# oasys-mas/free-range-zoo

Measured on NVIDIA B200. Metric: env-steps/sec, higher is better.
Workload: dtype int32+f32

## Files before the change

### __graft_entry__.py

```python
import os
import subprocess
import sys

ROOT = os.path.dirname(os.path.abspath(__file__))
if ROOT not in sys.path:
    sys.path.insert(0, ROOT)


def build() -> None:
    from oracle.build_ref import build_ref
    build_ref()
    from free_range_zoo_b200 import _build
    path = _build.build(verbose=False)
    assert os.path.exists(path), path
    from free_range_zoo_b200 import _lib
    lib = _lib.library()
    missing = [name for header in ('frz.h', 'frz_obs.h', 'frz_autoreset.h') for name in _lib.exported_symbols(header)
               if not hasattr(lib, name)]
    if missing:
        raise RuntimeError(f'libfrz.so does not export {missing}')
    import free_range_zoo_b200.envs.wildfire_v0


def smoke() -> None:
    import numpy as np
    import torch

    from free_range_zoo_b200 import presets
    from free_range_zoo_b200.envs import wildfire_v0
    from oracle.wildfire import WildfireOracle

    B, steps = 64, 3
    config = presets.wildfire_large()
    env = wildfire_v0.parallel_env(parallel_envs=B, max_steps=10, configuration=config, device=torch.device('cuda:0'))
    env.reset(seed=0)
    oracle = WildfireOracle(config, B, 10)
    oracle.reset()
    rng = np.random.default_rng(0)
    for _ in range(steps):
        counts = oracle.agent_task_count
        k = np.minimum((rng.random(counts.shape) * (counts + 1)).astype(np.int64), counts)
        actions = np.stack([k, np.where(k == counts, -1, 0)], axis=2).astype(np.int32)
        u_field = rng.random((3, B, 10, 10), dtype=np.float32)
        u_agent = rng.random((5, B, 10), dtype=np.float32)
        oracle.step(actions, u_field, u_agent)
        env.unwrapped.inject_uniforms(torch.from_numpy(u_field), torch.from_numpy(u_agent))
        _, rewards, terminations, _, _ = env.step(torch.from_numpy(actions).cuda())
    state = env.state()
    assert np.array_equal(state.fires.cpu().numpy(), oracle.fires)
    assert np.array_equal(state.intensity.cpu().numpy(), oracle.intensity)
    assert np.array_equal(state.equipment.cpu().numpy(), oracle.equipment)
    got = np.stack([rewards[a].cpu().numpy() for a in env.agents], axis=1)
    assert np.allclose(got, oracle.rewards, rtol=1e-5, atol=1e-6)
    print('smoke ok: wildfire 10x10/10 agents, 64 envs x 3 steps bit-exact vs oracle (injected uniforms)')

    from tests import philox_ref
    B, seed = 300, 0xC0FFEE
    env = wildfire_v0.parallel_env(parallel_envs=B, max_steps=10, configuration=config, device=torch.device('cuda:0'))
    env.reset(seed=seed)
    raw = env.unwrapped
    oracle = WildfireOracle(config, B, 10)
    oracle.reset()
    for t in range(steps):
        actions = philox_ref.sampled_actions(7, t, np.arange(B), oracle.agent_task_count)
        raw.sample_actions(7)
        assert np.array_equal(raw._actions.cpu().numpy(), actions)
        oracle.step(actions, *philox_ref.wildfire_uniforms(seed, t, np.arange(B), 10, 10, 10))
        raw.step_all()
    state = raw.state()
    for name in ('fires', 'intensity', 'fuel', 'equipment', 'suppressants', 'capacity'):
        assert np.array_equal(getattr(state, name).cpu().numpy(), getattr(oracle, name)), name
    assert np.array_equal(raw._task_obs.cpu().numpy(), oracle.task_obs)
    assert np.array_equal(raw._agent_task_count.cpu().numpy(), oracle.agent_task_count)
    assert np.allclose(raw._rewards.cpu().numpy(), oracle.rewards, rtol=1e-5, atol=1e-6)
    raw.check_errors()
    print('smoke ok: Philox-mode kernel, 300 envs x 3 steps bit-exact vs oracle on host-Philox uniforms')


if __name__ == '__main__':
    build()
    if len(sys.argv) > 1 and sys.argv[1] == 'smoke':
        smoke()
```

### free_range_zoo_b200/_lib.py

```python
from __future__ import annotations

import ctypes as C
import os

import torch

_HERE = os.path.dirname(os.path.abspath(__file__))
LIBRARY_PATH = os.environ.get('FRZ_LIBRARY') or os.path.join(_HERE, 'csrc', 'libfrz.so')

MAX_AGENTS = 32
MAX_EQUIPMENT = 8
MAX_CAPACITIES = 8
MAX_CELLS = 256
MAX_NODES = 32
MAX_NET_STATES = 16
MAX_PASSENGERS = 64
PAD = -100

FAULT_NAMES = {
    0x1: 'action[:, 0] is not a valid index into the agent\'s task list',
    0x2: 'cybersecurity attack / movement target outside [0, num_nodes)',
    0x4: 'a non-present cybersecurity agent acted while show_bad_actions=False',
    0x8: 'rideshare passenger table overflow',
}


class Control(C.Structure):
    _fields_ = [('seed', C.c_uint64), ('step', C.c_uint64), ('ctas_done', C.c_uint32), ('alive_acc', C.c_uint32),
                ('alive', C.c_uint32), ('error_word', C.c_uint32), ('agents_with_tasks_acc', C.c_uint32),
                ('agents_with_tasks', C.c_uint32), ('reserved', C.c_uint32 * 6)]


WF_FLAGS = dict(suppressant_decrease=0x0001, suppressant_refill=0x0002, tank_switch=0x0004, critical_error=0x0008,
                degrade=0x0010, repair=0x0020, fire_increase=0x0040, fire_decrease=0x0080,
                special_burnout_probability=0x0100, fire_fuel=0x0200)
WF_BURNOUT_SCALED = 0x0400
WF_LOCALIZE_PUTOUTS = 0x0800
WF_SHOW_BAD_ACTIONS = 0x1000
WF_KERNEL_TILES, WF_KERNEL_GROUPS = 0x2000, 0x4000


class WildfireParams(C.Structure):
    _fields_ = [
        ('height', C.c_int32), ('width', C.c_int32), ('num_agents', C.c_int32), ('num_fire_states', C.c_int32),
        ('num_equipment_states', C.c_int32), ('num_capacities', C.c_int32), ('max_steps', C.c_int32),
        ('flags', C.c_uint32), ('env_offset', C.c_int64),
        ('p_increase', C.c_float), ('p_burnout', C.c_float), ('p_decrease', C.c_float), ('decrease_bonus', C.c_float),
        ('p_random_ignition', C.c_float), ('spread_lut', C.c_float * 16),
        ('p_suppressant_decrease', C.c_float), ('p_refill', C.c_float), ('p_repair', C.c_float),
        ('p_degrade', C.c_float), ('p_critical', C.c_float), ('p_tank_switch', C.c_float),
        ('capacity_cum', C.c_float * MAX_CAPACITIES), ('capacity_value', C.c_float * MAX_CAPACITIES),
        ('equipment_capacity_bonus', C.c_float * MAX_EQUIPMENT), ('equipment_power_bonus', C.c_float * MAX_EQUIPMENT),
        ('bad_attack_penalty', C.c_float), ('burnout_penalty', C.c_float), ('termination_reward', C.c_float),
        ('termination_kappa', C.c_float),
        ('agent_y', C.c_int32 * MAX_AGENTS), ('agent_x', C.c_int32 * MAX_AGENTS), ('agent_power', C.c_float * MAX_AGENTS),
    ]


_WF_POINTERS = ('fires', 'intensity', 'fuel', 'suppressants', 'capacity', 'equipment', 'init_fires', 'init_intensity',
                'init_fuel', 'init_suppressants', 'init_capacity', 'init_equipment', 'actions', 'rewards',
                'cumulative_rewards', 'terminated', 'truncated', 'num_moves', 'num_burnouts', 'burnouts', 'putouts',
                'env_task_count', 'agent_task_count', 'action_mask', 'self_obs', 'task_obs', 'cell_reward',
                'cell_ignition', 'range_mask', 'cell_agents', 'control', 'field_uniforms', 'agent_uniforms')


class WildfireBuffers(C.Structure):
    _fields_ = [(name, C.c_void_p) for name in _WF_POINTERS] + [('mask_stride', C.c_int32), ('mask_words', C.c_int32)]


CY_STOCHASTIC_STATE = 0x1
CY_SHOW_BAD_ACTIONS = 0x2
CY_MAX_LUT_BITS = 12


class CyberParams(C.Structure):
    _fields_ = [
        ('num_nodes', C.c_int32), ('num_attackers', C.c_int32), ('num_defenders', C.c_int32), ('num_states', C.c_int32),
        ('max_steps', C.c_int32), ('flags', C.c_uint32), ('env_offset', C.c_int64), ('lut_bits', C.c_int32),
        ('temperature', C.c_float), ('patch_reward', C.c_float), ('bad_action_penalty', C.c_float),
        ('power', C.c_float * MAX_AGENTS), ('persist', C.c_float * MAX_AGENTS), ('returns', C.c_float * MAX_AGENTS),
        ('state_rewards', C.c_float * MAX_NET_STATES), ('criticality', C.c_float * MAX_NODES),
    ]


_CY_POINTERS = ('network_state', 'location', 'presence', 'init_network_state', 'init_location', 'init_presence',
                'actions', 'rewards', 'cumulative_rewards', 'terminated', 'truncated', 'num_moves', 'env_task_count',
                'agent_task_count', 'attacker_self', 'defender_self', 'task_obs', 'monitored', 'score_lut', 'control',
                'network_uniforms', 'agent_uniforms')


class CyberBuffers(C.Structure):
    _fields_ = [(name, C.c_void_p) for name in _CY_POINTERS]


RS_FAST_TRAVEL = 0x1
RS_DIAGONAL_TRAVEL = 0x2
RS_VARIABLE_MOVE_COST = 0x4
RS_WAITING_COSTS = 0x8
RS_KERNEL_TILES, RS_KERNEL_GROUPS = 0x100, 0x200
RS_PASSENGER_COLUMNS = 11
RS_TASK_COLUMNS = 8


class RideshareParams(C.Structure):
    _fields_ = [
        ('num_agents', C.c_int32), ('capacity', C.c_int32), ('schedule_rows', C.c_int32), ('schedule_horizon', C.c_int32),
        ('pool_limit', C.c_int32),
        ('max_steps', C.c_int32), ('flags', C.c_uint32), ('env_offset', C.c_int64), ('wait_limit', C.c_int32 * 3),
        ('long_wait_time', C.c_int32), ('move_cost', C.c_float), ('drop_cost', C.c_float), ('noop_cost', C.c_float),
        ('accept_cost', C.c_float), ('pool_limit_cost', C.c_float), ('general_wait_cost', C.c_float),
        ('long_wait_cost', C.c_float),
    ]


_RS_POINTERS = ('agents', 'passengers', 'init_agents', 'init_passengers', 'init_count', 'schedule', 'schedule_index', 'actions',
                'rewards', 'cumulative_rewards', 'terminated', 'truncated', 'num_moves', 'env_task_count',
                'agent_task_count', 'task_mask', 'self_obs', 'task_obs', 'control')


class RideshareBuffers(C.Structure):
    _fields_ = [(name, C.c_void_p) for name in _RS_POINTERS]


MAX_CHUNKS = 16


class HostStep(C.Structure):
    _fields_ = [('actions', C.c_void_p), ('rewards', C.c_void_p), ('terminated', C.c_void_p), ('truncated', C.c_void_p),
                ('chunk_controls', C.c_void_p), ('streams', C.POINTER(C.c_void_p)), ('chunks', C.c_int32),
                ('action_format', C.c_int32), ('packed_actions', C.c_void_p), ('pipeline', C.c_void_p)]


class GatherArray(C.Structure):
    _fields_ = [('src', C.c_void_p), ('dst', C.c_void_p), ('row_bytes', C.c_int32), ('capacity', C.c_int32),
                ('groups', C.c_int32), ('reserved', C.c_int32)]


class ObsArray(C.Structure):
    _fields_ = [('src', C.c_void_p), ('dst', C.c_void_p), ('host', C.c_void_p), ('kind', C.c_int32), ('src_type', C.c_int32),
                ('dst_type', C.c_int32), ('groups', C.c_int32), ('capacity', C.c_int32), ('src_columns', C.c_int32),
                ('column_first', C.c_int32), ('columns', C.c_int32)]


class ObsDownload(C.Structure):
    _fields_ = [('counts', C.c_void_p), ('offsets', C.c_void_p), ('host_offsets', C.c_void_p), ('scan', C.c_void_p),
                ('scratch', C.c_void_p),
                ('status', C.c_void_p), ('arrays', C.POINTER(ObsArray)), ('array_count', C.c_int32),
                ('mask_groups', C.c_int32)]


class AutoresetRow(C.Structure):
    _fields_ = [('dst', C.c_void_p), ('src', C.c_void_p), ('bytes', C.c_int64)]


AUTORESET_MAX_ROWS = 32


class Autoreset(C.Structure):
    _fields_ = [(name, C.c_void_p) for name in (
        'terminated', 'truncated', 'step_terminated', 'step_truncated', 'done', 'cumulative_rewards', 'episode_return',
        'num_moves', 'episode_length', 'agent_task_count', 'reset_agent_task_count', 'control', 'finished',
        'finished_count', 'scratch')] + [('rows', C.POINTER(AutoresetRow)), ('row_count', C.c_int32),
                                         ('num_agents', C.c_int32)]


OBS_DENSE, OBS_ROWS, OBS_MASK_BITS = 0, 1, 2
OBS_I32, OBS_I16, OBS_I8, OBS_U8, OBS_F32 = 0, 1, 2, 3, 4
HOST_ACTIONS_I32, HOST_ACTIONS_I16, HOST_ACTIONS_I8 = 0, 1, 2
ABI_VERSION = 4


_lib = None


def library() -> C.CDLL:
    global _lib
    if _lib is not None:
        return _lib
    if not os.path.exists(LIBRARY_PATH):
        raise RuntimeError(f'{LIBRARY_PATH} is missing: the B200 engine has no CPU fallback. '
                           'Build it with `python -c "import __graft_entry__ as g; g.build()"`.')
    lib = C.CDLL(LIBRARY_PATH)
    lib.frz_version.restype = C.c_int
    lib.frz_last_error.restype = C.c_char_p
    lib.frz_control_init.argtypes = [C.c_void_p, C.c_uint64, C.c_void_p]
    for name in ('frz_wildfire_step', 'frz_wildfire_refresh'):
        getattr(lib, name).argtypes = [C.POINTER(WildfireParams), C.POINTER(WildfireBuffers), C.c_int32, C.c_void_p]
    lib.frz_wildfire_reset.argtypes = [C.POINTER(WildfireParams), C.POINTER(WildfireBuffers), C.c_int32, C.c_void_p,
                                       C.c_void_p]
    lib.frz_wildfire_sample_actions.argtypes = [C.POINTER(WildfireParams), C.POINTER(WildfireBuffers), C.c_int32,
                                                C.c_uint64, C.c_void_p]
    for name in ('frz_cyber_step', 'frz_cyber_refresh'):
        getattr(lib, name).argtypes = [C.POINTER(CyberParams), C.POINTER(CyberBuffers), C.c_int32, C.c_void_p]
    lib.frz_cyber_reset.argtypes = [C.POINTER(CyberParams), C.POINTER(CyberBuffers), C.c_int32, C.c_void_p, C.c_void_p]
    lib.frz_cyber_sample_actions.argtypes = [C.POINTER(CyberParams), C.POINTER(CyberBuffers), C.c_int32, C.c_uint64,
                                             C.c_void_p]
    for name in ('frz_rideshare_step', 'frz_rideshare_refresh'):
        getattr(lib, name).argtypes = [C.POINTER(RideshareParams), C.POINTER(RideshareBuffers), C.c_int32, C.c_void_p]
    lib.frz_rideshare_reset.argtypes = [C.POINTER(RideshareParams), C.POINTER(RideshareBuffers), C.c_int32, C.c_void_p,
                                        C.c_void_p]
    lib.frz_rideshare_sample_actions.argtypes = [C.POINTER(RideshareParams), C.POINTER(RideshareBuffers), C.c_int32,
                                                 C.c_uint64, C.c_void_p]
    for name, params, buffers in (('frz_wildfire_step_host', WildfireParams, WildfireBuffers),
                                  ('frz_cyber_step_host', CyberParams, CyberBuffers),
                                  ('frz_rideshare_step_host', RideshareParams, RideshareBuffers)):
        getattr(lib, name).argtypes = [C.POINTER(params), C.POINTER(buffers), C.c_int32, C.POINTER(HostStep), C.c_void_p]
    lib.frz_host_slices.argtypes = [C.c_int32, C.c_int32, C.POINTER(C.c_int32)]
    lib.frz_wildfire_tile_random_layout.argtypes = [C.POINTER(WildfireParams), C.POINTER(C.c_uint32), C.POINTER(C.c_int8)]
    lib.frz_gather_live_rows.argtypes = [C.c_void_p, C.c_int32, C.c_void_p, C.c_void_p, C.POINTER(GatherArray), C.c_int32,
                                         C.c_void_p]
    lib.frz_observe_compact.argtypes = [C.POINTER(ObsDownload), C.c_int32, C.c_void_p]
    lib.frz_autoreset.argtypes = [C.POINTER(Autoreset), C.c_int32, C.c_void_p]
    if lib.frz_version() != ABI_VERSION:
        raise RuntimeError(f'libfrz.so ABI version {lib.frz_version()} != {ABI_VERSION}; rebuild the library')
    lib.frz_control_restore.argtypes = [C.c_void_p, C.c_uint64, C.c_uint64, C.c_void_p]
    lib.frz_host_pipeline_create.argtypes = [C.POINTER(C.c_void_p)]
    lib.frz_host_pipeline_destroy.argtypes = [C.c_void_p]
    for name, params in (('frz_wildfire_buffer_bytes', WildfireParams), ('frz_cyber_buffer_bytes', CyberParams),
                         ('frz_rideshare_buffer_bytes', RideshareParams)):
        getattr(lib, name).argtypes = [C.POINTER(params), C.c_int32, C.c_char_p]
        getattr(lib, name).restype = C.c_int64
    _lib = lib
    return lib


def host_slices(parallel_envs: int, chunks: int):
    bounds = (C.c_int32 * (MAX_CHUNKS + 1))()
    count = library().frz_host_slices(parallel_envs, chunks, bounds)
    if count < 0:
        check(-count, 'frz_host_slices')
    return list(bounds[:count + 1])


def check(status: int, what: str = '') -> None:
    if status != 0:
        message = library().frz_last_error().decode()
        raise RuntimeError(f'libfrz {what} failed (status {status}): {message}')


def stream_handle(device: torch.device) -> C.c_void_p:
    return C.c_void_p(torch.cuda.current_stream(device).cuda_stream)


def pointer(tensor: torch.Tensor | None) -> int | None:
    return None if tensor is None else tensor.data_ptr()


def exported_symbols(header: str = 'frz.h'):
    import re
    header = os.path.join(os.path.dirname(_HERE), 'include', header)
    text = open(header).read()
    return sorted(set(re.findall(r'\b(frz_[a-z_]+)\s*\(', text)))
```

### free_range_zoo_b200/csrc/frz_common.cuh

```cuda
#pragma once

#include <cuda_runtime.h>
#include <stdint.h>

#include <vector>

#include "frz.h"

struct FrzHostPipeline {
  int device = -1;
  cudaEvent_t events[1 + 2 * FRZ_MAX_CHUNKS] = {};
  cudaGraph_t graph = nullptr;
  cudaGraphExec_t exec = nullptr;
  std::vector<unsigned char> signature;
  struct ActionCopy {
    cudaGraphNode_t node;
    void* dst;
    size_t offset, bytes;
  };
  std::vector<ActionCopy> action_copies;
  const void* captured_actions = nullptr;
};

namespace frz {

constexpr unsigned kFullMask = 0xffffffffu;
constexpr int kMaxDevices = 64;


void set_error(const char* fmt, ...);
int check_launch(const char* what);

inline int current_device() {
  int device = 0;
  cudaGetDevice(&device);
  return device;
}

inline int sm_count() {
  static int cache[kMaxDevices] = {};
  const int device = current_device();
  int count = (device >= 0 && device < kMaxDevices) ? cache[device] : 0;
  if (count == 0) {
    cudaDeviceGetAttribute(&count, cudaDevAttrMultiProcessorCount, device);
    if (count < 1) count = 1;
    if (device >= 0 && device < kMaxDevices) cache[device] = count;
  }
  return count;
}

template <class Kernel>
int resident_ctas(Kernel kernel, int threads, size_t smem) {
  static int ctas[kMaxDevices] = {};
  static size_t smem_of[kMaxDevices] = {};
  const int device = current_device();
  const bool cacheable = device >= 0 && device < kMaxDevices;
  if (cacheable && ctas[device] > 0 && smem_of[device] == smem) return ctas[device];
  int count = 0;
  cudaOccupancyMaxActiveBlocksPerMultiprocessor(&count, kernel, threads, smem);
  if (count < 1) count = 1;
  if (cacheable) {
    ctas[device] = count;
    smem_of[device] = smem;
  }
  return count;
}

inline int persistent_grid(int work_ctas, int ctas_per_sm) {
  const int cap = sm_count() * ctas_per_sm;
  return work_ctas < cap ? (work_ctas < 1 ? 1 : work_ctas) : cap;
}

int control_broadcast(FrzControl* main_block, FrzControl* chunk_blocks, int count, cudaStream_t stream);
int control_merge(FrzControl* main_block, FrzControl* chunk_blocks, int count, cudaStream_t stream);
cudaEvent_t* pipeline_events(FrzHostPipeline* pipeline);
int widen_actions(const void* packed, int element_bytes, int32_t* actions, size_t count, cudaStream_t stream);


struct Philox {
  uint32_t key0, key1;
  __device__ __forceinline__ Philox(uint64_t seed) : key0(uint32_t(seed)), key1(uint32_t(seed >> 32)) {}

  __device__ __forceinline__ uint4 operator()(uint32_t c0, uint32_t c1, uint32_t c2, uint32_t c3) const {
    uint32_t k0 = key0, k1 = key1;
#pragma unroll
    for (int round = 0; round < 10; ++round) {
      const uint32_t hi0 = __umulhi(0xD2511F53u, c0), lo0 = 0xD2511F53u * c0;
      const uint32_t hi1 = __umulhi(0xCD9E8D57u, c2), lo1 = 0xCD9E8D57u * c2;
      c0 = hi1 ^ c1 ^ k0;
      c1 = lo1;
      c2 = hi0 ^ c3 ^ k1;
      c3 = lo0;
      k0 += 0x9E3779B9u;
      k1 += 0xBB67AE85u;
    }
    return make_uint4(c0, c1, c2, c3);
  }
};

__device__ __forceinline__ float u01(uint32_t bits) { return float(bits >> 8) * 5.9604644775390625e-08f; }

__device__ __forceinline__ int select_bit(uint32_t w, int k) {
  int pos = 0;
#pragma unroll
  for (int span = 16; span >= 1; span >>= 1) {
    const int below = __popc(w & ((1u << span) - 1u));
    if (k >= below) {
      k -= below;
      w >>= span;
      pos += span;
    }
  }
  return pos;
}


__device__ __forceinline__ uint32_t shared_address(const void* pointer) {
  return static_cast<uint32_t>(__cvta_generic_to_shared(pointer));
}
__device__ __forceinline__ uint32_t lds_const(uint32_t address) {
  uint32_t value;
  asm("ld.shared.u32 %0, [%1];" : "=r"(value) : "r"(address));
  return value;
}
__device__ __forceinline__ uint4 lds_const_v4(uint32_t address) {
  uint4 value;
  asm("ld.shared.v4.u32 {%0, %1, %2, %3}, [%4];" : "=r"(value.x), "=r"(value.y), "=r"(value.z), "=r"(value.w) : "r"(address));
  return value;
}
__device__ __forceinline__ uint32_t lds(uint32_t address) {
  uint32_t value;
  asm volatile("ld.shared.u32 %0, [%1];" : "=r"(value) : "r"(address) : "memory");
  return value;
}
__device__ __forceinline__ uint4 lds_v4(uint32_t address) {
  uint4 value;
  asm volatile("ld.shared.v4.u32 {%0, %1, %2, %3}, [%4];"
               : "=r"(value.x), "=r"(value.y), "=r"(value.z), "=r"(value.w) : "r"(address) : "memory");
  return value;
}
__device__ __forceinline__ void sts(uint32_t address, uint32_t value) {
  asm volatile("st.shared.u32 [%0], %1;" : : "r"(address), "r"(value) : "memory");
}

__device__ __forceinline__ void cp_async_4(uint32_t shared_dst, const void* global_src) {
  asm volatile("cp.async.ca.shared.global [%0], [%1], 4;" : : "r"(shared_dst), "l"(global_src) : "memory");
}
__device__ __forceinline__ void cp_async_8(uint32_t shared_dst, const void* global_src) {
  asm volatile("cp.async.ca.shared.global [%0], [%1], 8;" : : "r"(shared_dst), "l"(global_src) : "memory");
}
__device__ __forceinline__ void cp_async_16(uint32_t shared_dst, const void* global_src) {
  asm volatile("cp.async.cg.shared.global [%0], [%1], 16;" : : "r"(shared_dst), "l"(global_src) : "memory");
}
__device__ __forceinline__ void cp_async_commit() { asm volatile("cp.async.commit_group;" : : : "memory"); }
__device__ __forceinline__ void cp_async_wait_all() { asm volatile("cp.async.wait_group 0;" : : : "memory"); }


__device__ __forceinline__ bool elect_one() {
  uint32_t elected;
  asm volatile(
      "{\n"
      ".reg .pred p;\n"
      "elect.sync _|p, 0xffffffff;\n"
      "selp.u32 %0, 1, 0, p;\n"
      "}\n"
      : "=r"(elected));
  return elected != 0u;
}

__device__ __forceinline__ void mbarrier_init(uint32_t barrier, uint32_t arrivals) {
  asm volatile("mbarrier.init.shared::cta.b64 [%0], %1;" : : "r"(barrier), "r"(arrivals) : "memory");
  asm volatile("fence.mbarrier_init.release.cluster;" : : : "memory");
}
__device__ __forceinline__ void mbarrier_expect_bytes(uint32_t barrier, uint32_t bytes) {
  asm volatile("mbarrier.arrive.expect_tx.shared::cta.b64 _, [%0], %1;" : : "r"(barrier), "r"(bytes) : "memory");
}
__device__ __forceinline__ void mbarrier_arrive(uint32_t barrier) {
  asm volatile("mbarrier.arrive.shared::cta.b64 _, [%0];" : : "r"(barrier) : "memory");
}
__device__ __forceinline__ void named_barrier_sync(int id, int threads) {
  asm volatile("bar.sync %0, %1;" : : "r"(id), "r"(threads) : "memory");
}
__device__ __forceinline__ void mbarrier_wait(uint32_t barrier, uint32_t parity) {
  asm volatile(
      "{\n"
      ".reg .pred done;\n"
      "WAIT_LOOP:\n"
      "mbarrier.try_wait.parity.shared::cta.b64 done, [%0], %1;\n"
      "@!done bra WAIT_LOOP;\n"
      "}\n"
      : : "r"(barrier), "r"(parity) : "memory");
}
__device__ __forceinline__ void bulk_load(uint32_t shared_dst, const void* global_src, uint32_t bytes, uint32_t barrier) {
  asm volatile("cp.async.bulk.shared::cluster.global.mbarrier::complete_tx::bytes [%0], [%1], %2, [%3];"
               : : "r"(shared_dst), "l"(global_src), "r"(bytes), "r"(barrier) : "memory");
}
__device__ __forceinline__ void bulk_store(void* global_dst, uint32_t shared_src, uint32_t bytes) {
  asm volatile("cp.async.bulk.global.shared::cta.bulk_group [%0], [%1], %2;"
               : : "l"(global_dst), "r"(shared_src), "r"(bytes) : "memory");
}
__device__ __forceinline__ void bulk_commit() { asm volatile("cp.async.bulk.commit_group;" : : : "memory"); }
__device__ __forceinline__ void bulk_wait_read() { asm volatile("cp.async.bulk.wait_group.read 0;" : : : "memory"); }
template <int pending>
__device__ __forceinline__ void bulk_wait_read_all_but() {
  asm volatile("cp.async.bulk.wait_group.read %0;" : : "n"(pending) : "memory");
}
__device__ __forceinline__ void fence_async_shared() { asm volatile("fence.proxy.async.shared::cta;" : : : "memory"); }


enum Publish { kPublishNothing = 0, kPublishRefresh = 1, kPublishStep = 2 };

__device__ __forceinline__ void finish_launch(FrzControl* control, unsigned alive_bits, unsigned fault_bits,
                                              unsigned agent_bits, int publish) {
  __shared__ unsigned s_alive, s_fault, s_agents;
  if (threadIdx.x == 0) {
    s_alive = 0;
    s_fault = 0;
    s_agents = 0;
  }
  __syncthreads();
  if (alive_bits) atomicOr(&s_alive, alive_bits);
  if (fault_bits) atomicOr(&s_fault, fault_bits);
  if (agent_bits) atomicOr(&s_agents, agent_bits);
  __syncthreads();
  if (threadIdx.x == 0) {
    if (s_alive) atomicOr(&control->alive_acc, s_alive);
    if (s_fault) atomicOr(&control->error_word, s_fault);
    if (s_agents) atomicOr(&control->agents_with_tasks_acc, s_agents);
    __threadfence();
    const unsigned arrived = atomicAdd(&control->ctas_done, 1u) + 1u;
    if (arrived == gridDim.x) {
      __threadfence();
      const unsigned alive = atomicExch(&control->alive_acc, 0u);
      const unsigned agents = atomicExch(&control->agents_with_tasks_acc, 0u);
      if (publish == kPublishStep) {
        control->alive = alive;
        control->step += 1;
      }
      if (publish != kPublishNothing) control->agents_with_tasks = agents;
      if (publish == kPublishRefresh) control->alive = alive;
      control->ctas_done = 0u;
    }
  }
}

}
```

### free_range_zoo_b200/csrc/frz_wildfire.cu

```cuda
#include <cmath>
#include <math_constants.h>

#include "frz_common.cuh"
#include "frz_host.cuh"

namespace frz {
namespace {

#ifndef FRZ_WF_THREADS
#define FRZ_WF_THREADS 256
#endif
constexpr int kThreads = FRZ_WF_THREADS;
enum Mode { kStep = 0, kRefresh = 1 };

template <int NW>
__device__ __forceinline__ uint32_t word_at(const uint32_t (&words)[NW], int index) {
  uint32_t w = words[0];
#pragma unroll
  for (int i = 1; i < NW; ++i) w = (index == i) ? words[i] : w;
  return w;
}

template <int NW>
__device__ __forceinline__ bool bit_at(const uint32_t (&words)[NW], int cell) {
  return (word_at<NW>(words, cell >> 5) >> (cell & 31)) & 1u;
}

template <int G>
__device__ __forceinline__ float group_sum(float v) {
#pragma unroll
  for (int offset = G / 2; offset >= 1; offset >>= 1) v += __shfl_xor_sync(kFullMask, v, offset, G);
  return v;
}

template <int G>
__device__ __forceinline__ int group_sum(int v) {
#pragma unroll
  for (int offset = G / 2; offset >= 1; offset >>= 1) v += __shfl_xor_sync(kFullMask, v, offset, G);
  return v;
}

template <int G>
__device__ __forceinline__ uint32_t group_ballot(bool pred, int group_base, uint32_t group_mask) {
  const uint32_t ballot = __ballot_sync(kFullMask, pred);
  return (G == 32) ? ballot : ((ballot >> group_base) & group_mask);
}

#ifndef FRZ_WF_CELLS_IN_SMEM
#define FRZ_WF_CELLS_IN_SMEM 1
#endif
__host__ __device__ constexpr bool split_geometry(int group, int cells_per_lane) { return group == 16 && cells_per_lane > 4; }
__host__ __device__ constexpr bool cells_in_smem(int group, int cells_per_lane) {
  return FRZ_WF_CELLS_IN_SMEM && split_geometry(group, cells_per_lane);
}
__host__ __device__ constexpr int group_smem_words(int group, int cells_per_lane) {
  const int cells = group * cells_per_lane;
  const int words = cells_in_smem(group, cells_per_lane) ? 8 * cells + 5 * group : 2 * cells;
  return (group == 16 && words % 32 == 0) ? words + 16 : words;
}
__host__ __device__ inline int static_smem_words(int cells, int agents, int states) {
  const int words = (cells + 31) / 32;
  return 4 * cells + states * cells + agents * states * words;
}

template <int G, int CPL, int NW>
__device__ __forceinline__ void assemble_words(const uint32_t (&rows)[CPL], uint32_t (&words)[NW], int group_base,
                                               uint32_t group_mask, uint32_t half_selector) {
  if constexpr (G == 32) {
#pragma unroll
    for (int i = 0; i < CPL; ++i) words[i] = rows[i];
  } else if constexpr (CPL == 1) {
    words[0] = (rows[0] >> group_base) & group_mask;
  } else if constexpr (G == 16) {
#pragma unroll
    for (int w = 0; w < NW; ++w) words[w] = __byte_perm(rows[2 * w], (2 * w + 1 < CPL) ? rows[(2 * w + 1 < CPL) ? 2 * w + 1 : 0] : 0u, half_selector);
  } else {
    static_assert(G == 8 && CPL <= 4, "8-lane groups hold at most 4 cells per lane");
    const uint32_t lo = __byte_perm(rows[0], rows[1], half_selector);
    const uint32_t hi = CPL > 2 ? __byte_perm(rows[2], rows[CPL - 1], half_selector) : 0u;
    uint32_t word = __byte_perm(lo, hi, 0x5410);
    if (CPL == 2) word &= 0xffffu;
    if (CPL == 3) word &= 0xffffffu;
    words[0] = word;
  }
}

template <int NW>
__device__ __forceinline__ void load_range_words(uint32_t address, uint32_t (&words)[NW]) {
  if constexpr (NW == 4) {
    const uint4 v = lds_const_v4(address);
    words[0] = v.x;
    words[1] = v.y;
    words[2] = v.z;
    words[3] = v.w;
  } else {
#pragma unroll
    for (int w = 0; w < NW; ++w) words[w] = lds_const(address + 4u * w);
  }
}

#ifndef FRZ_WF_MIN_BLOCKS
#define FRZ_WF_MIN_BLOCKS 3
#endif

struct Derived {
  uint32_t west_ok[FRZ_MAX_CELLS / 32];
  uint32_t east_ok[FRZ_MAX_CELLS / 32];
  int32_t spare_lanes_feed_agents;
  uint32_t t_increase, t_burnout, t_suppressant_decrease, t_repair, t_critical, t_degrade, t_refill, t_tank_switch;
  int32_t t_capacity_cum[FRZ_MAX_CAPACITIES];
  int32_t almost_state, burned_state;
  int32_t cells;
};

template <int G, int CPL, int MODE, bool INJECTED, bool BULK>
__global__ void __launch_bounds__(kThreads, (G * CPL > 128) ? 1 : FRZ_WF_MIN_BLOCKS)
wildfire_step_kernel(const __grid_constant__ FrzWildfireParams p, const __grid_constant__ FrzWildfireBuffers io,
                     const __grid_constant__ Derived derived, const int B) {
  constexpr int mode = MODE;
  constexpr int kGroupsPerWarp = 32 / G;
  constexpr int kCells = G * CPL;
  constexpr int NW = (kCells + 31) / 32;
  constexpr int kCalls = (2 * CPL + 3) / 4;
  static_assert(G == 32 || G == 16 || CPL <= 4, "8-lane groups hold at most four cells per lane (one mask word)");
  constexpr int RPW = (CPL == 1) ? 1 : 32 / G;
  constexpr int kFullRows = (G == 32) ? CPL / 2 : (CPL - 1);
  extern __shared__ __align__(16) uint32_t smem[];

  const int lane = threadIdx.x & 31;
  const int warp_in_cta = __shfl_sync(kFullMask, int(threadIdx.x >> 5), 0);
  const int sub = lane % G;
  const int group_base = lane - sub;
  const uint32_t group_mask = (G == 32) ? 0xffffffffu : ((1u << G) - 1u);
  uint32_t lane_bit = 1u << sub;
  asm volatile("" : "+r"(lane_bit));
  const auto row_bit = [&](int i) { return lane_bit << ((i % RPW) * G); };
  const uint32_t half_selector = (G == 16) ? ((group_base & 16) ? 0x7632u : 0x5410u)
                                           : (uint32_t(group_base >> 3) | ((4u + uint32_t(group_base >> 3)) << 4));
  const int W = p.width, HW = derived.cells;
  const int A = p.num_agents;
  const int E = p.num_equipment_states;
  const uint32_t flags = p.flags;
  const bool show_bad = flags & FRZ_WF_SHOW_BAD_ACTIONS;
  const bool use_fuel = flags & FRZ_WF_FIRE_FUEL;
  const int mask_words_row = io.mask_stride >> 2;
  const int table_words = io.mask_words;

  constexpr int kYOff = 0, kXOff = kCells, kIgnitionOff = 2 * kCells, kRewardOff = 3 * kCells, kRegionOff = 4 * kCells;
  constexpr int kCellAgentsOff = kRegionOff + (kThreads / 32) * kGroupsPerWarp * group_smem_words(G, CPL);
  constexpr bool kCellsInSmem = cells_in_smem(G, CPL);
  const int range_off = kCellAgentsOff + E * kCells;
  const int attack_off = kRegionOff + (warp_in_cta * kGroupsPerWarp + lane / G) * group_smem_words(G, CPL);
  const int tasks_off = attack_off + kCells;
  const uint32_t s_base = shared_address(smem);
  uint32_t s_cell = s_base + 4u * uint32_t(sub);
  asm volatile("" : "+r"(s_cell));
  uint32_t s_attack = s_base + 4u * uint32_t(attack_off);
  asm volatile("" : "+r"(s_attack));
  const uint32_t s_tasks = s_base + 4u * uint32_t(tasks_off);
  const uint32_t s_range = s_base + 4u * uint32_t(range_off);
  uint32_t* my_state = smem + tasks_off + kCells + sub;
  constexpr bool bulk = BULK;
  static_assert(!BULK || kCellsInSmem, "the bulk path moves the shared-memory state planes");
  const uint32_t s_barriers = s_base + 4u * uint32_t((range_off + A * E * NW + 3) & ~3) + 16u * uint32_t(warp_in_cta);
  const uint32_t s_planes = s_base + 4u * uint32_t(tasks_off + kCells);
  const auto planes_of_group = [&](int g) {
    return s_base + 4u * uint32_t(kRegionOff + (warp_in_cta * kGroupsPerWarp + g) * group_smem_words(G, CPL) + 2 * kCells);
  };
  constexpr uint32_t kBufferBytes = 4u * 3u * kCells;
  const uint32_t s_stage = s_planes + 2u * kBufferBytes + 4u * uint32_t(sub);

  for (int i = threadIdx.x; i < E * kCells; i += kThreads) {
    const int e = i / kCells, c = i - e * kCells;
    smem[kCellAgentsOff + i] = c < HW ? io.cell_agents[e * HW + c] : 0u;
  }
  for (int i = threadIdx.x; i < A * E * NW; i += kThreads) {
    const int row = i / NW, w = i - row * NW;
    smem[range_off + i] = w < table_words ? io.range_mask[row * table_words + w] : 0u;
  }
  for (int c = threadIdx.x; c < kCells; c += kThreads) {
    const int y = c / W, x = c - y * W;
    const bool in_grid = c < HW;
    smem[kYOff + c] = uint32_t(y);
    smem[kXOff + c] = uint32_t(x);
    smem[kIgnitionOff + c] = in_grid ? uint32_t(io.cell_ignition[c]) : 0u;
    smem[kRewardOff + c] = in_grid ? __float_as_uint(io.cell_reward[c]) : 0u;
  }
#pragma unroll
  for (int i = 0; i < CPL; ++i) smem[attack_off + i * G + sub] = 0u;
  if constexpr (kCellsInSmem) {
#pragma unroll
    for (int i = 0; i < 6 * CPL; ++i) my_state[i * G] = 0u;
    if (bulk && lane == 0) {
      mbarrier_init(s_barriers, 1);
      mbarrier_init(s_barriers + 8u, 1);
    }
  }
  __syncthreads();

  FrzControl* const control = io.control;
  const uint64_t step = control->step;
  const uint32_t alive_prev = control->alive;
  const uint32_t agents_with_tasks = control->agents_with_tasks;
  const Philox philox(control->seed);
  const bool skip = (mode == kStep) && ((alive_prev & 3u) != 3u);

  const bool is_agent = sub < A;
  const float base_power = is_agent ? p.agent_power[sub] : 0.f;
  const float agent_yf = is_agent ? float(p.agent_y[sub]) : 0.f;
  const float agent_xf = is_agent ? float(p.agent_x[sub]) : 0.f;

  unsigned alive_bits = 0, faults = 0, agent_bits = 0;

  if (!skip) {
    const int groups_per_cta = (kThreads / 32) * kGroupsPerWarp;
    const int first_env0 = (blockIdx.x * (kThreads / 32) + warp_in_cta) * kGroupsPerWarp;
    const uint32_t row_bytes = 4u * uint32_t(HW);
    const auto fetch_state = [&](int pair, uint32_t into) {
      const uint32_t buffer = __shfl_sync(kFullMask, into, 0);
      if (elect_one()) {
        const uint32_t barrier = s_barriers + 8u * buffer;
        mbarrier_expect_bytes(barrier, uint32_t(kGroupsPerWarp) * 3u * row_bytes);
#pragma unroll
        for (int g = 0; g < kGroupsPerWarp; ++g) {
          const size_t at = size_t(min(pair + g, B - 1)) * size_t(HW);
          const uint32_t planes = planes_of_group(g) + kBufferBytes * buffer;
          bulk_load(planes, io.fires + at, row_bytes, barrier);
          bulk_load(planes + 4u * kCells, io.intensity + at, row_bytes, barrier);
          bulk_load(planes + 8u * kCells, io.fuel + at, row_bytes, barrier);
        }
      }
      if (is_agent) {
        const uint32_t at = uint32_t(min(pair + lane / G, B - 1)) * uint32_t(A) + uint32_t(sub);
        cp_async_4(s_stage, io.suppressants + at);
        cp_async_4(s_stage + 4u * G, io.capacity + at);
        cp_async_4(s_stage + 8u * G, io.equipment + at);
        if (mode == kStep) cp_async_8(s_stage + 12u * G + 4u * uint32_t(sub), io.actions + 2u * at);
      }
      cp_async_commit();
    };
    uint32_t buffer = 0u, parities = 0u;
    if constexpr (kCellsInSmem) {
      if (bulk && first_env0 < B) fetch_state(first_env0, 0u);
    }
    for (int env0 = first_env0; env0 < B; env0 += gridDim.x * groups_per_cta) {
      const int env = env0 + lane / G;
      const bool valid = (G == 32) || env < B;
      const int e = valid ? env : B - 1;
      const uint32_t cell_row = uint32_t(e) * uint32_t(HW);
      const uint32_t agent_at = uint32_t(e) * uint32_t(A) + uint32_t(sub);
      int* const fires_row = io.fires + cell_row;
      int* const inten_row = io.intensity + cell_row;
      int* const fuel_row = io.fuel + cell_row;

      int cell_regs[3][kCellsInSmem ? 1 : CPL] = {};
      const auto cell = [&](int plane, int i) -> int {
        if constexpr (kCellsInSmem) return int(my_state[plane * kCells + i * G]);
        else return cell_regs[plane][i];
      };
      const auto set_cell = [&](int plane, int i, int value) {
        if constexpr (kCellsInSmem) my_state[plane * kCells + i * G] = uint32_t(value);
        else cell_regs[plane][i] = value;
      };
      uint32_t litw[NW], rows[CPL];
      if constexpr (bulk) {
        mbarrier_wait(s_barriers + 8u * buffer, (parities >> buffer) & 1u);
        parities ^= 1u << buffer;
#pragma unroll
        for (int i = 0; i < CPL; ++i) rows[i] = __ballot_sync(kFullMask, cell(0, i) > 0);
      } else {
#pragma unroll
        for (int i = 0; i < CPL; ++i) {
          const int c = i * G + sub;
          const bool in_grid = i < kFullRows || c < HW;
          const int f = in_grid ? fires_row[c] : 0;
          set_cell(0, i, f);
          set_cell(1, i, in_grid ? inten_row[c] : 0);
          set_cell(2, i, in_grid ? fuel_row[c] : 0);
          rows[i] = __ballot_sync(kFullMask, f > 0);
        }
      }
      float supp = 0.f, cap = 0.f;
      int equip = 0;
      int2 staged_action = make_int2(0, -1);
      if constexpr (bulk) {
        cp_async_wait_all();
        if (is_agent) {
          supp = __uint_as_float(lds(s_stage));
          cap = __uint_as_float(lds(s_stage + 4u * G));
          equip = min(max(int(lds(s_stage + 8u * G)), 0), E - 1);
          if (mode == kStep) {
            staged_action.x = int(lds(s_stage + 12u * G + 4u * uint32_t(sub)));
            staged_action.y = int(lds(s_stage + 12u * G + 4u * uint32_t(sub) + 4u));
          }
        }
      } else if (is_agent) {
        supp = io.suppressants[agent_at];
        cap = io.capacity[agent_at];
        equip = min(max(io.equipment[agent_at], 0), E - 1);
      }

      int n_before = 0;
      assemble_words<G, CPL, NW>(rows, litw, group_base, group_mask, half_selector);
#pragma unroll
      for (int w = 0; w < NW; ++w) n_before += __popc(litw[w]);
      if (mode != kStep) n_before = HW;

      float reward = 0.f, cumulative = 0.f;
      int moves = 0, total_burnouts = 0, n_burned = 0, n_putout = 0;
      bool terminated = false, truncated = false;

      const auto prefetch_next = [&]() {
        if constexpr (kCellsInSmem) {
          const int next_env0 = env0 + gridDim.x * groups_per_cta;
          if (bulk && next_env0 < B) {
            if (lane == 0) bulk_wait_read();
            fetch_state(next_env0, buffer ^ 1u);
          }
        }
      };
      if (mode != kStep) prefetch_next();

      if (mode == kStep) {
        int act_k = 0, act_id = -1;
        if (is_agent) {
          const int2 act = bulk ? staged_action : reinterpret_cast<const int2*>(io.actions)[agent_at];
          act_k = act.x;
          act_id = act.y;
          cumulative = io.cumulative_rewards[agent_at];
        }
        moves = io.num_moves[e];
        total_burnouts = io.num_burnouts[e];
        const bool was_terminated = io.terminated[e] != 0;

        const bool refill = is_agent && act_id == -1;
        int target = -1;
        bool bad = false;
        if (is_agent && !refill && ((agents_with_tasks >> sub) & 1u)) {
          uint32_t availw[NW];
          load_range_words<NW>(s_range + 4u * uint32_t((sub * E + equip) * NW), availw);
#pragma unroll
          for (int w = 0; w < NW; ++w) availw[w] = supp > 0.f ? (litw[w] & availw[w]) : 0u;
          int k = act_k, found = -1, base_bit = 0;
          uint32_t chosen = 0u;
          bool hit = false;
          if (k >= 0) {
#pragma unroll
            for (int w = 0; w < NW; ++w) {
              const uint32_t choices = show_bad ? litw[w] : availw[w];
              const int count = __popc(choices);
              if (!hit) {
                if (k < count) {
                  hit = true;
                  chosen = choices;
                  base_bit = 32 * w;
                } else {
                  k -= count;
                }
              }
            }
          }
          if (hit) found = base_bit + select_bit(chosen, k);
          if (found < 0) faults |= FRZ_FAULT_BAD_TASK_INDEX;
          else if (show_bad && !bit_at<NW>(availw, found)) bad = true;
          else target = found;
        }
        const bool user = target >= 0;
        const float power = base_power + p.equipment_power_bonus[equip];

        {
          const uint32_t key = user ? (uint32_t(group_base) << 16 | uint32_t(target)) : (0x80000000u | uint32_t(lane));
          uint32_t peers = __match_any_sync(kFullMask, key);
          if (!user) peers = 0u;
          float total = 0.f;
          while (__any_sync(kFullMask, peers != 0u)) {
            const int source = (__ffs(peers) - 1) & 31;
            const float theirs = __shfl_sync(kFullMask, power, source);
            if (peers != 0u) total = __fadd_rn(total, theirs);
            peers &= peers - 1u;
          }
          if (user) sts(s_attack + 4u * uint32_t(target), __float_as_uint(total));
          __syncwarp();
        }

        constexpr bool kSplit = !INJECTED && split_geometry(G, CPL) && 2 * ((CPL + 3) / 4) == kCalls;
        constexpr int kCallsA = kSplit ? kCalls / 2 : kCalls;
        const auto grow_word = [](int i) { return kSplit ? i : 2 * i; };
        const auto spread_word = [](int i) { return kSplit ? 4 * kCallsA + i : 2 * i + 1; };
        float ua[5], uf[INJECTED ? 3 * CPL : 1];
        uint32_t ka[5];
        uint32_t bits[4 * kCalls];
        const bool inject_agent = INJECTED && io.agent_uniforms != nullptr;
        const bool inject_field = INJECTED && io.field_uniforms != nullptr;
        const uint32_t env_lo = uint32_t(p.env_offset + e), env_hi = uint32_t(uint64_t(p.env_offset + e) >> 32);
        const uint32_t step_lo = uint32_t(step), step_hi = uint32_t(step >> 32) ^ env_hi;
        const auto draw = [&](int first_call, int last_call) {
#pragma unroll
          for (int k = first_call; k < last_call; ++k) {
            const uint4 r = philox(env_lo, step_lo, uint32_t(k * G + sub), step_hi);
            bits[4 * k] = r.x;
            bits[4 * k + 1] = r.y;
            bits[4 * k + 2] = r.z;
            bits[4 * k + 3] = r.w;
          }
        };
        if (!inject_field || !inject_agent) draw(0, kCallsA);
        if constexpr (INJECTED) {
          const size_t plane = size_t(B) * HW;
#pragma unroll
          for (int i = 0; i < CPL; ++i) {
            const int c = i * G + sub;
            if (inject_field) {
#pragma unroll
              for (int ev = 0; ev < 3; ++ev) uf[3 * i + ev] = c < HW ? io.field_uniforms[ev * plane + cell_row + c] : 1.f;
            } else {
              uf[3 * i] = uf[3 * i + 1] = u01(bits[grow_word(i)]);
              uf[3 * i + 2] = u01(bits[spread_word(i)]);
            }
          }
        }
        const auto field_uniform = [&](int i, int event) -> float {
          if constexpr (INJECTED) return uf[3 * i + event];
          else return u01(bits[event == 2 ? spread_word(i) : grow_word(i)]);
        };

        const auto agent_phase = [&]() {
          if (inject_agent) {
#pragma unroll
            for (int ev = 0; ev < 5; ++ev)
              ua[ev] = is_agent ? io.agent_uniforms[(size_t(ev) * B + e) * A + sub] : 1.f;
          } else {
            uint32_t words[4];
            bool have_words = false;
            constexpr int kSpareOwn = 4 * kCalls - 2 * CPL;
            constexpr int kOwnA = kSplit ? CPL : 2 * CPL, kOwnB = kSplit ? 4 * kCallsA + CPL : 2 * CPL + 1;
            if constexpr (CPL > 1) {
              if (derived.spare_lanes_feed_agents) {
                const int first = group_base + ((G - 1 - sub) & (G - 1)), second = group_base + ((G - 1 - A - sub) & (G - 1));
                const uint32_t a = __shfl_sync(kFullMask, bits[grow_word(CPL - 1)], first);
                const uint32_t b = __shfl_sync(kFullMask, bits[spread_word(CPL - 1)], first);
                if constexpr (kSpareOwn == 2) {
                  words[0] = bits[kOwnA < 4 * kCalls ? kOwnA : 0];
                  words[1] = bits[kOwnB < 4 * kCalls ? kOwnB : 0];
                  words[2] = a;
                  words[3] = b;
                } else {
                  words[0] = a;
                  words[1] = b;
                  words[2] = __shfl_sync(kFullMask, bits[grow_word(CPL - 1)], second);
                  words[3] = __shfl_sync(kFullMask, bits[spread_word(CPL - 1)], second);
                }
                have_words = true;
              }
            }
            if (!have_words) {
              const uint4 r = philox(env_lo, step_lo, 0x80000000u | uint32_t(sub), step_hi);
              words[0] = r.x;
              words[1] = r.y;
              words[2] = r.z;
              words[3] = r.w;
            }
            if constexpr (INJECTED) {
              ua[0] = ua[2] = u01(words[0]);
              ua[1] = u01(words[1]);
              ua[3] = u01(words[2]);
              ua[4] = u01(words[3]);
            } else {
              ka[0] = ka[2] = words[0] >> 8;
              ka[1] = words[1] >> 8;
              ka[3] = words[2] >> 8;
              ka[4] = words[3] >> 8;
            }
          }
          const auto happens = [&](int ev, float p_event, uint32_t t_event) -> bool {
            if constexpr (INJECTED) return ua[ev] < p_event;
            else return ka[ev] < t_event;
          };

          const bool decrease = user && happens(0, p.p_suppressant_decrease, derived.t_suppressant_decrease);
          supp = fmaxf(decrease ? __fadd_rn(supp, -1.f) : supp, 0.f);
          {
            const bool pristine = equip == E - 1, damaged = equip == 0;
            const bool wearable = pristine || !damaged;
            const bool repairs = damaged && happens(1, p.p_repair, derived.t_repair);
            const bool critical = pristine && happens(1, p.p_critical, derived.t_critical);
            const bool degrades = wearable && happens(1, p.p_degrade, derived.t_degrade) && !critical;
            if (repairs) equip = E - 1;
            if (critical) equip = 0;
            if (degrades) equip -= 1;
          }
          const bool increased = refill && happens(2, p.p_refill, derived.t_refill);
          if (increased) supp = __fadd_rn(cap, p.equipment_capacity_bonus[max(equip, 0)]);
          if (__any_sync(kFullMask, increased)) {
            int pick = 0;
#pragma unroll
            for (int i = 0; i < FRZ_MAX_CAPACITIES; ++i) {
              if constexpr (INJECTED) pick += ua[3] > p.capacity_cum[i] ? 1 : 0;
              else pick += int(ka[3]) > derived.t_capacity_cum[i] ? 1 : 0;
            }
            pick = min(pick, p.num_capacities - 1);
            const bool switches = increased && happens(4, p.p_tank_switch, derived.t_tank_switch);
            const float extra = __fadd_rn(supp, -cap);
            if (switches) {
              cap = p.capacity_value[pick];
              supp = __fadd_rn(cap, extra);
            }
          }
        };
        if constexpr (!kSplit) agent_phase();

        uint32_t burned_bits = 0, putout_bits = 0;
        uint32_t burnw[NW];
#pragma unroll
        for (int i = 0; i < CPL; ++i) {
          const float attack = __uint_as_float(lds(s_attack + 4u * uint32_t(i * G + sub)));
          int f = cell(0, i), it = cell(1, i);
          const bool burning = f > 0 && it > 0;
          const float diff = __fadd_rn(f > 0 ? float(f) : 0.f, -attack);
          const bool unmet = burning && diff > 0.f;
          bool grow;
          float u_down;
          if constexpr (INJECTED) {
            u_down = field_uniform(i, 1);
            grow = unmet && field_uniform(i, 0) < (it == derived.almost_state ? p.p_burnout : p.p_increase);
          } else {
            const uint32_t k24 = bits[grow_word(i)] >> 8;
            u_down = float(k24) * 5.9604644775390625e-08f;
            grow = unmet && (it == derived.almost_state ? k24 < derived.t_burnout : k24 < derived.t_increase);
          }
          it += grow ? 1 : 0;
          const bool burned = grow && it >= derived.burned_state;
          const bool met = burning && !burned && diff <= 0.f;
          const float prob_down = fminf(fmaxf(__fadd_rn(p.p_decrease, __fmul_rn(-diff, p.decrease_bonus)), 0.f), 1.f);
          const bool shrink = met && u_down < prob_down;
          it -= shrink ? 1 : 0;
          const bool put = shrink && it <= 0;
          if (burned || put) {
            const int fuel = cell(2, i) - 1;
            set_cell(2, i, burned ? max(fuel, 0) : fuel);
            f = -f;
          }
          burned_bits |= uint32_t(burned) << i;
          putout_bits |= uint32_t(put) << i;
          if (!kCellsInSmem || burned || put) set_cell(0, i, f);
          if (!kCellsInSmem || grow || shrink) set_cell(1, i, it);
          rows[i] = __ballot_sync(kFullMask, burning && !burned && !put);
        }
        assemble_words<G, CPL, NW>(rows, burnw, group_base, group_mask, half_selector);
        __syncwarp();
        if (user) sts(s_attack + 4u * uint32_t(target), 0u);

        if constexpr (kSplit) draw(kCallsA, kCalls);
        prefetch_next();
#pragma unroll
        for (int w = 0; w < NW; ++w) {
          int f[RPW], it[RPW];
          bool unlit[RPW], any_unlit = false;
#pragma unroll
          for (int r = 0; r < RPW; ++r) {
            const int i = w * RPW + r;
            unlit[r] = false;
            if (i < CPL) {
              f[r] = cell(0, i);
              it[r] = cell(1, i);
              unlit[r] = f[r] < 0 && it[r] == 0 && (!use_fuel || cell(2, i) > 0);
              any_unlit = any_unlit || unlit[r];
            }
          }
          if (__any_sync(kFullMask, any_unlit)) {
            const uint32_t cur = burnw[w];
            const uint32_t prev = w > 0 ? burnw[w > 0 ? w - 1 : 0] : 0u;
            const uint32_t next = w + 1 < NW ? burnw[w + 1 < NW ? w + 1 : 0] : 0u;
            uint32_t north, south;
            if (W < 32) {
              north = __funnelshift_l(prev, cur, W);
              south = __funnelshift_r(cur, next, W);
            } else {
              const int q = W >> 5, r = W & 31;
              const auto word_or_zero = [&](int v) { return (v >= 0 && v < NW) ? word_at<NW>(burnw, v) : 0u; };
              north = __funnelshift_l(word_or_zero(w - q - 1), word_or_zero(w - q), r);
              south = __funnelshift_r(word_or_zero(w + q), word_or_zero(w + q + 1), r);
            }
            const uint32_t west = __funnelshift_l(prev, cur, 1) & derived.west_ok[w];
            const uint32_t east = __funnelshift_r(cur, next, 1) & derived.east_ok[w];
#pragma unroll
            for (int r = 0; r < RPW; ++r) {
              const int i = w * RPW + r;
              if (i < CPL) {
                const uint32_t my_bit = row_bit(i);
                float prob = 0.f;
                if (north & my_bit) prob = p.spread_lut[1];
                if (west & my_bit) prob = __fadd_rn(prob, p.spread_lut[2]);
                if (east & my_bit) prob = __fadd_rn(prob, p.spread_lut[4]);
                if (south & my_bit) prob = __fadd_rn(prob, p.spread_lut[8]);
                prob = __fadd_rn(prob, p.p_random_ignition);
                if (unlit[r] && field_uniform(i, 2) < prob) {
                  f[r] = -f[r];
                  it[r] = int(lds_const(s_cell + 4u * (kIgnitionOff + i * G)));
                  if (kCellsInSmem) {
                    set_cell(0, i, f[r]);
                    set_cell(1, i, it[r]);
                  }
                }
              }
            }
          }
#pragma unroll
          for (int r = 0; r < RPW; ++r) {
            const int i = w * RPW + r;
            if (i < CPL) {
              if (!kCellsInSmem) {
                set_cell(0, i, f[r]);
                set_cell(1, i, it[r]);
              }
              rows[i] = __ballot_sync(kFullMask, f[r] > 0);
            }
          }
        }
        assemble_words<G, CPL, NW>(rows, litw, group_base, group_mask, half_selector);

        if constexpr (kSplit) agent_phase();

        if constexpr (G == 32) {
          n_burned = __reduce_add_sync(kFullMask, __popc(burned_bits));
          n_putout = __reduce_add_sync(kFullMask, __popc(putout_bits));
        } else {
          n_burned = group_sum<G>(__popc(burned_bits));
          n_putout = group_sum<G>(__popc(putout_bits));
        }
        float put_total = 0.f, burn_total = 0.f;
        uint32_t putw[NW];
#pragma unroll
        for (int w = 0; w < NW; ++w) putw[w] = 0u;
        const bool localize = flags & FRZ_WF_LOCALIZE_PUTOUTS, scaled = flags & FRZ_WF_BURNOUT_SCALED;
        if (__any_sync(kFullMask, n_putout != 0) && !localize) {
          float my_put_reward = 0.f;
#pragma unroll
          for (int i = 0; i < CPL; ++i)
            if ((putout_bits >> i) & 1u) my_put_reward += __uint_as_float(lds_const(s_cell + 4u * (kRewardOff + i * G)));
          put_total = group_sum<G>(my_put_reward);
        }
        if (__any_sync(kFullMask, n_putout != 0) && localize) {
#pragma unroll
          for (int i = 0; i < CPL; ++i) rows[i] = __ballot_sync(kFullMask, (putout_bits >> i) & 1u);
          assemble_words<G, CPL, NW>(rows, putw, group_base, group_mask, half_selector);
        }
        if (__any_sync(kFullMask, n_burned != 0) && scaled) {
          float my_burn_reward = 0.f;
#pragma unroll
          for (int i = 0; i < CPL; ++i)
            if ((burned_bits >> i) & 1u) my_burn_reward += __uint_as_float(lds_const(s_cell + 4u * (kRewardOff + i * G)));
          burn_total = group_sum<G>(my_burn_reward);
        }
        const float penalty_total =
            (flags & FRZ_WF_BURNOUT_SCALED) ? -burn_total : __fmul_rn(p.burnout_penalty, float(n_burned));
        uint32_t any_lit = 0;
#pragma unroll
        for (int w = 0; w < NW; ++w) any_lit |= litw[w];
        bool dead = any_lit == 0;
        if (use_fuel && __any_sync(kFullMask, dead)) {
          int my_fuel = 0;
#pragma unroll
          for (int i = 0; i < CPL; ++i) my_fuel += cell(2, i);
          const int fuel_left = group_sum<G>(my_fuel);
          dead = dead && fuel_left <= 0;
        }
        if (dead) {
#pragma unroll
          for (int i = 0; i < CPL; ++i) set_cell(0, i, 0);
#pragma unroll
          for (int w = 0; w < NW; ++w) litw[w] = 0;
        }
        const bool newly = !was_terminated && dead;
        terminated = was_terminated || dead;
        reward = bad ? p.bad_attack_penalty : 0.f;
        float gain = put_total;
        if (flags & FRZ_WF_LOCALIZE_PUTOUTS)
          gain = (target >= 0 && bit_at<NW>(putw, target)) ? __uint_as_float(lds_const(s_base + 4u * uint32_t(kRewardOff + target))) : 0.f;
        reward = __fadd_rn(reward, __fadd_rn(gain, penalty_total));
        if (newly) {
          const float penalty = __fmul_rn(p.termination_kappa, logf(__fadd_rn(float(total_burnouts), 1.f)));
          reward = __fadd_rn(reward, fmaxf(__fadd_rn(p.termination_reward, -penalty), 0.f));
        }
        total_burnouts += n_burned;
        moves += 1;
        truncated = moves >= p.max_steps;
        cumulative = __fadd_rn(cumulative, reward);
        if (valid) alive_bits |= (terminated ? 0u : 1u) | (truncated ? 0u : 2u);
      } else if (valid) {
        alive_bits |= (io.terminated[e] ? 0u : 1u) | (io.truncated[e] ? 0u : 2u);
      }

      if constexpr (G != 32) {
        if (!valid) {
          n_before = 0;
#pragma unroll
          for (int w = 0; w < NW; ++w) litw[w] = 0u;
        }
      }
      int n_lit = 0;
#pragma unroll
      for (int w = 0; w < NW; ++w) n_lit += __popc(litw[w]);
      const int n_rows = max(n_lit, n_before);

      int n_avail = 0;
      if (is_agent && supp > 0.f) {
        uint32_t reach[NW];
        load_range_words<NW>(s_range + 4u * uint32_t((sub * E + max(equip, 0)) * NW), reach);
#pragma unroll
        for (int w = 0; w < NW; ++w) n_avail += __popc(litw[w] & reach[w]);
      }
      uint32_t fighters[CPL];
#pragma unroll
      for (int i = 0; i < CPL; ++i) fighters[i] = 0u;
      for (int q = 0; q < E; ++q) {
        const uint32_t ready = group_ballot<G>(is_agent && supp > 0.f && equip == q, group_base, group_mask);
#pragma unroll
        for (int i = 0; i < CPL; ++i) fighters[i] |= lds_const(s_cell + 4u * uint32_t(kCellAgentsOff + q * kCells + i * G)) & ready;
      }
      int4* const task_rows = reinterpret_cast<int4*>(io.task_obs);
      {
        int rank = 0;
#pragma unroll
        for (int i = 0; i < CPL; ++i) {
          const uint32_t word = litw[i / RPW], my_bit = row_bit(i);
          if (i > 0 && i % RPW == 0) rank += __popc(litw[i > 0 ? i / RPW - 1 : 0]);
          if (word & my_bit) {
            const int t = rank + __popc(word & (my_bit - 1u));
            sts(s_tasks + 4u * uint32_t(t), fighters[i]);
            task_rows[cell_row + uint32_t(t)] = make_int4(int(lds_const(s_cell + 4u * (kYOff + i * G))), int(lds_const(s_cell + 4u * (kXOff + i * G))),
                                      cell(0, i), cell(1, i));
          }
        }
      }
      const int quads = (n_rows + 3) >> 2;
      const int quads_warp = __reduce_max_sync(kFullMask, quads);
      for (int first = n_lit; first < 4 * quads; first += G) {
        const int t = first + sub;
        if (t < 4 * quads) {
          sts(s_tasks + 4u * uint32_t(t), 0u);
          if (t < n_before) task_rows[cell_row + uint32_t(t)] = make_int4(FRZ_PAD, FRZ_PAD, FRZ_PAD, FRZ_PAD);
        }
      }
      __syncwarp();

      if (valid) {
        uint32_t* const mask_words = reinterpret_cast<uint32_t*>(io.action_mask);
        const uint32_t mask_env = uint32_t(env) * uint32_t(A) * uint32_t(mask_words_row);
        const int span_shift = min(32 - __clz(max(quads_warp, 1) - 1), (G == 32) ? 5 : (G == 16) ? 4 : 3);
        const int span = 1 << span_shift, slots = G >> span_shift;
        const int slot = sub >> span_shift, quad_in_span = sub & (span - 1);
        for (int first = 0; first < quads; first += span) {
          const int q = first + quad_in_span;
          if (q < quads) {
            const uint4 m = lds_v4(s_tasks + 16u * uint32_t(q));
            constexpr int kPlanes = G / 8;
            uint32_t at = mask_env + uint32_t(slot * mask_words_row + q);
            const uint32_t stride = uint32_t(slots * mask_words_row);
            int a = slot;
#pragma unroll
            for (int k = 0; k < kPlanes; ++k) {
              if (k > 0 && 8 * k >= A) break;
              const uint32_t selector = uint32_t(k | ((4 + k) << 4));
              const uint32_t plane = __byte_perm(__byte_perm(m.x, m.y, selector), __byte_perm(m.z, m.w, selector), 0x5410);
              const int end = min(A, 8 * k + 8);
              for (; a < end; a += slots, at += stride) mask_words[at] = (plane >> (a & 7)) & 0x01010101u;
            }
          }
        }

        if (is_agent) {
          io.agent_task_count[agent_at] = n_avail;
          if (n_avail > 0) agent_bits |= lane_bit;
          reinterpret_cast<float4*>(io.self_obs)[agent_at] =
              make_float4(agent_yf, agent_xf, base_power, supp);
        }
        if (sub == 0) io.env_task_count[env] = n_lit;

        if (mode == kStep) {
          if (!bulk) {
#pragma unroll
            for (int i = 0; i < CPL; ++i) {
              const int c = i * G + sub;
              if (i < kFullRows || c < HW) {
                fires_row[c] = cell(0, i);
                inten_row[c] = cell(1, i);
                fuel_row[c] = cell(2, i);
              }
            }
          }
          if (is_agent) {
            io.suppressants[agent_at] = supp;
            io.capacity[agent_at] = cap;
            io.equipment[agent_at] = equip;
            io.rewards[agent_at] = reward;
            io.cumulative_rewards[agent_at] = cumulative;
          }
          if (sub == 0) {
            io.terminated[env] = terminated;
            io.truncated[env] = truncated;
            io.num_moves[env] = moves;
            io.num_burnouts[env] = total_burnouts;
            io.burnouts[env] = n_burned;
            io.putouts[env] = n_putout;
          }
        }
      }
      if constexpr (kCellsInSmem) {
        if (bulk) {
          if (mode == kStep) {
            fence_async_shared();
            __syncwarp();
            const uint32_t from = __shfl_sync(kFullMask, buffer, 0);
            if (lane == 0) {
#pragma unroll
              for (int g = 0; g < kGroupsPerWarp; ++g) {
                if (env0 + g < B) {
                  const size_t at = size_t(env0 + g) * size_t(HW);
                  const uint32_t planes = planes_of_group(g) + kBufferBytes * from;
                  bulk_store(io.fires + at, planes, row_bytes);
                  bulk_store(io.intensity + at, planes + 4u * kCells, row_bytes);
                  bulk_store(io.fuel + at, planes + 8u * kCells, row_bytes);
                }
              }
              bulk_commit();
            }
          }
          buffer ^= 1u;
          my_state = smem + tasks_off + kCells + sub + buffer * (3 * kCells);
        }
      }
      __syncwarp();
    }
    if constexpr (kCellsInSmem) {
      if (bulk && lane == 0) bulk_wait_read();
    }
  }
  finish_launch(control, alive_bits, faults, agent_bits,
                skip ? kPublishNothing : (mode == kStep ? kPublishStep : kPublishRefresh));
}


__global__ void wildfire_restore_kernel(const FrzWildfireParams p, const FrzWildfireBuffers io, const int B,
                                        const uint8_t* __restrict__ env_mask) {
  const int HW = p.height * p.width, A = p.num_agents;
  const int per_env = HW > A ? HW : A;
  const size_t total = size_t(B) * per_env;
  for (size_t i = size_t(blockIdx.x) * blockDim.x + threadIdx.x; i < total; i += size_t(gridDim.x) * blockDim.x) {
    const int env = int(i / per_env), j = int(i % per_env);
    if (env_mask != nullptr && !env_mask[env]) continue;
    if (j < HW) {
      const size_t at = size_t(env) * HW + j;
      io.fires[at] = io.init_fires[at];
      io.intensity[at] = io.init_intensity[at];
      io.fuel[at] = io.init_fuel[at];
    }
    if (j < A) {
      const size_t at = size_t(env) * A + j;
      io.suppressants[at] = io.init_suppressants[at];
      io.capacity[at] = io.init_capacity[at];
      io.equipment[at] = io.init_equipment[at];
      io.rewards[at] = 0.f;
      io.cumulative_rewards[at] = 0.f;
    }
    if (j == 0) {
      io.terminated[env] = 0;
      io.truncated[env] = 0;
      io.num_moves[env] = 0;
      io.num_burnouts[env] = 0;
      io.burnouts[env] = 0;
      io.putouts[env] = 0;
    }
  }
}

__global__ void wildfire_sample_kernel(const FrzWildfireParams p, const FrzWildfireBuffers io, const int B,
                                       const uint64_t sampler_seed) {
  const int A = p.num_agents;
  const Philox philox(sampler_seed);
  const uint64_t step = io.control->step;
  const bool show_bad = p.flags & FRZ_WF_SHOW_BAD_ACTIONS;
  const int total = B * A;
  for (int i = blockIdx.x * blockDim.x + threadIdx.x; i < total; i += gridDim.x * blockDim.x) {
    const int env = i / A, agent = i - env * A;
    const int n = show_bad ? io.env_task_count[env] : io.agent_task_count[i];
    const uint64_t genv = uint64_t(p.env_offset + env);
    const uint4 r = philox(uint32_t(genv), uint32_t(step), 0xC0000000u | uint32_t(agent), uint32_t(step >> 32) ^ uint32_t(genv >> 32));
    const int k = min(int(u01(r.x) * float(n + 1)), n);
    reinterpret_cast<int2*>(const_cast<int32_t*>(io.actions))[i] = make_int2(k, k == n ? -1 : 0);
  }
}

#ifndef FRZ_WF_HALF_WARP_CELLS
#define FRZ_WF_HALF_WARP_CELLS 128
#endif

struct Geometry {
  int group, cells_per_lane;
};

bool pick_geometry(const FrzWildfireParams& p, Geometry* g) {
  const int HW = p.height * p.width, A = p.num_agents;
  if (A < 1 || A > FRZ_MAX_AGENTS || HW < 1 || HW > FRZ_MAX_CELLS) return false;
  if (HW <= 8 && A <= 8) *g = {8, 1};
  else if (HW <= 32 && A <= 8) *g = {8, (HW + 7) / 8};
  else if (HW <= 16 && A <= 16) *g = {16, 1};
  else if (HW <= FRZ_WF_HALF_WARP_CELLS && A <= 16) *g = {16, (HW + 15) / 16};
  else if (HW <= 32) *g = {32, 1};
  else if (HW <= 64) *g = {32, 2};
  else if (HW <= 128) *g = {32, 4};
  else *g = {32, 8};
  return true;
}

void fold_configuration(const FrzWildfireParams& in, int group, int cells_per_lane, FrzWildfireParams* out, Derived* derived) {
  *out = in;
  const uint32_t flags = in.flags;
  const auto clamp01 = [](float v) { return v < 0.f ? 0.f : (v > 1.f ? 1.f : v); };
  if (!(flags & FRZ_WF_STOCH_SUPPRESSANT_DECREASE)) out->p_suppressant_decrease = 2.f;
  if (!(flags & FRZ_WF_STOCH_REFILL)) out->p_refill = 2.f;
  if (!(flags & FRZ_WF_STOCH_TANK_SWITCH)) out->p_tank_switch = 2.f;
  if (!(flags & FRZ_WF_CRITICAL_ERROR)) out->p_critical = -1.f;
  if (!(flags & FRZ_WF_STOCH_DEGRADE)) out->p_degrade = 2.f;
  if (!(flags & FRZ_WF_STOCH_REPAIR)) out->p_repair = 2.f;
  out->p_increase = (flags & FRZ_WF_STOCH_FIRE_INCREASE) ? clamp01(in.p_increase) : 1.f;
  out->p_burnout = clamp01((flags & FRZ_WF_SPECIAL_BURNOUT) ? in.p_burnout : in.p_increase);
  if (!(flags & FRZ_WF_STOCH_FIRE_DECREASE)) {
    out->p_decrease = 2.f;
    out->decrease_bonus = 0.f;
  }
  for (int i = in.num_capacities; i < FRZ_MAX_CAPACITIES; ++i) out->capacity_cum[i] = INFINITY;
  const int H = in.height, W = in.width, HW = H * W;
  for (int w = 0; w < FRZ_MAX_CELLS / 32; ++w) derived->west_ok[w] = derived->east_ok[w] = 0u;
  for (int c = 0; c < HW; ++c) {
    const int x = c % W;
    if (x > 0) derived->west_ok[c >> 5] |= 1u << (c & 31);
    if (x < W - 1) derived->east_ok[c >> 5] |= 1u << (c & 31);
  }
  {
    const auto below = [](float probability) {
      const double scaled = std::ceil(double(probability) * 16777216.0);
      return uint32_t(scaled < 0.0 ? 0.0 : (scaled > 16777216.0 ? 16777216.0 : scaled));
    };
    derived->t_increase = below(out->p_increase);
    derived->t_burnout = below(out->p_burnout);
    derived->t_suppressant_decrease = below(out->p_suppressant_decrease);
    derived->t_repair = below(out->p_repair);
    derived->t_critical = below(out->p_critical);
    derived->t_degrade = below(out->p_degrade);
    derived->t_refill = below(out->p_refill);
    derived->t_tank_switch = below(out->p_tank_switch);
    for (int i = 0; i < FRZ_MAX_CAPACITIES; ++i) {
      const double scaled = std::floor(double(out->capacity_cum[i]) * 16777216.0);
      derived->t_capacity_cum[i] = std::isnan(scaled) ? (1 << 24) : int32_t(scaled < -1.0 ? -1.0 : (scaled > 16777216.0 ? 16777216.0 : scaled));
    }
    derived->almost_state = in.num_fire_states - 2;
    derived->burned_state = in.num_fire_states - 1;
    derived->cells = in.height * in.width;
  }
  derived->spare_lanes_feed_agents = 0;
  if (cells_per_lane > 1) {
    const int last_row_cells = HW - group * (cells_per_lane - 1);
    const int spare_lanes = group - (last_row_cells > 0 ? last_row_cells : 0);
    const int calls = (2 * cells_per_lane + 3) / 4, spare_own = 4 * calls - 2 * cells_per_lane;
    const int lanes_needed = spare_own == 2 ? in.num_agents : 2 * in.num_agents;
    derived->spare_lanes_feed_agents = lanes_needed <= spare_lanes ? 1 : 0;
  }
}

#include "frz_wildfire_tile.cuh"

template <int MAXA, int MODE, bool INJECTED>
int launch_tiles(const FrzWildfireParams& caller_params, const FrzWildfireBuffers& io, int B, const Geometry& g,
                 cudaStream_t stream) {
  FrzWildfireParams p;
  Derived derived;
  fold_configuration(caller_params, g.group, g.cells_per_lane, &p, &derived);
  const SmallRandomLayout layout = small_random_layout(p.height * p.width, p.num_agents, g.group, g.cells_per_lane,
                                                       derived.spare_lanes_feed_agents != 0);
  const size_t smem = size_t(small_tile(p.height * p.width, p.num_agents).total) * sizeof(uint32_t);
  auto kernel = wildfire_tile_kernel<MAXA, MODE, INJECTED>;
  if (smem > 48 * 1024 && cudaFuncSetAttribute(kernel, cudaFuncAttributeMaxDynamicSharedMemorySize, int(smem)) != cudaSuccess)
    return check_launch("wildfire tile shared memory");
  cudaFuncSetAttribute(kernel, cudaFuncAttributePreferredSharedMemoryCarveout, cudaSharedmemCarveoutMaxShared);
  const int tiles = (B + 31) / 32;
  const int resident = sm_count() * resident_ctas(kernel, 32, smem);
  const int rounds = (tiles + resident - 1) / resident;
  const int grid = (tiles + rounds - 1) / rounds;
  kernel<<<grid, 32, smem, stream>>>(p, io, derived, layout, B);
  return check_launch("wildfire_tile_kernel");
}

template <int MAXA>
int launch_tiles_mode(const FrzWildfireParams& p, const FrzWildfireBuffers& io, int B, int mode, const Geometry& g,
                      cudaStream_t stream) {
  if (mode != kStep) return launch_tiles<MAXA, kRefresh, false>(p, io, B, g, stream);
  if (io.field_uniforms != nullptr || io.agent_uniforms != nullptr) return launch_tiles<MAXA, kStep, true>(p, io, B, g, stream);
  return launch_tiles<MAXA, kStep, false>(p, io, B, g, stream);
}

template <int G, int CPL, int MODE, bool INJECTED, bool BULK>
int launch_variant(const FrzWildfireParams& caller_params, const FrzWildfireBuffers& io, int B, cudaStream_t stream) {
  FrzWildfireParams p;
  Derived derived;
  fold_configuration(caller_params, G, CPL, &p, &derived);
  const int groups_per_cta = (kThreads / 32) * (32 / G);
  const size_t smem = (size_t(static_smem_words(G * CPL, p.num_agents, p.num_equipment_states)) +
                       size_t(groups_per_cta) * group_smem_words(G, CPL)) * sizeof(uint32_t) +
                      (BULK ? 16 + 16 * (kThreads / 32) : 0);
  auto kernel = wildfire_step_kernel<G, CPL, MODE, INJECTED, BULK>;
  if (smem > 48 * 1024) {
    if (cudaFuncSetAttribute(kernel, cudaFuncAttributeMaxDynamicSharedMemorySize, int(smem)) != cudaSuccess)
      return check_launch("wildfire smem attribute");
  }
  const int grid = persistent_grid((B + groups_per_cta - 1) / groups_per_cta, resident_ctas(kernel, kThreads, smem));
  kernel<<<grid, kThreads, smem, stream>>>(p, io, derived, B);
  return check_launch("wildfire_step_kernel");
}

template <int G, int CPL, bool BULK>
int launch_mode(const FrzWildfireParams& p, const FrzWildfireBuffers& io, int B, int mode, cudaStream_t stream) {
  if (mode != kStep) return launch_variant<G, CPL, kRefresh, false, BULK>(p, io, B, stream);
  if (io.field_uniforms != nullptr || io.agent_uniforms != nullptr) return launch_variant<G, CPL, kStep, true, BULK>(p, io, B, stream);
  return launch_variant<G, CPL, kStep, false, BULK>(p, io, B, stream);
}

template <int G, int CPL>
int launch_step(const FrzWildfireParams& p, const FrzWildfireBuffers& io, int B, int mode, cudaStream_t stream) {
  if constexpr (cells_in_smem(G, CPL)) {
    const uintptr_t bases = reinterpret_cast<uintptr_t>(io.fires) | reinterpret_cast<uintptr_t>(io.intensity) |
                            reinterpret_cast<uintptr_t>(io.fuel);
    if ((p.height * p.width) % 4 == 0 && bases % 16 == 0) return launch_mode<G, CPL, true>(p, io, B, mode, stream);
  }
  return launch_mode<G, CPL, false>(p, io, B, mode, stream);
}

int dispatch(const FrzWildfireParams* p, const FrzWildfireBuffers* io, int B, int mode, void* stream) {
  if (p == nullptr || io == nullptr || io->control == nullptr || io->fires == nullptr || io->cell_agents == nullptr ||
      io->range_mask == nullptr) {
    set_error("frz_wildfire: NULL params / buffers");
    return FRZ_ERR_NULL;
  }
  Geometry g;
  if (B <= 0 || !pick_geometry(*p, &g) || p->num_equipment_states < 1 || p->num_equipment_states > FRZ_MAX_EQUIPMENT ||
      p->num_capacities < 1 || p->num_capacities > FRZ_MAX_CAPACITIES || io->mask_stride % 4 != 0 ||
      io->mask_stride < p->height * p->width) {
    set_error("frz_wildfire: unsupported shape B=%d H=%d W=%d A=%d E=%d", B, p->height, p->width, p->num_agents,
              p->num_equipment_states);
    return FRZ_ERR_SHAPE;
  }
  {
    const uint64_t cells = uint64_t(B) * uint64_t(p->height * p->width);
    const uint64_t mask_words = uint64_t(B) * uint64_t(p->num_agents) * uint64_t(io->mask_stride / 4);
    if (cells >= (1ull << 32) || mask_words >= (1ull << 32)) {
      set_error("frz_wildfire: B=%d is too large for one launch (arrays exceed 2^32 elements); shard the batch", B);
      return FRZ_ERR_SHAPE;
    }
  }
  cudaStream_t s = static_cast<cudaStream_t>(stream);
  if (small_grid(*p) && g.group == 8 &&
      ((p->flags & FRZ_WF_KERNEL_TILES) ||
       (!(p->flags & FRZ_WF_KERNEL_GROUPS) && tiny_grid(*p) && B >= kSmallTileMinimumBatch))) {
    return p->num_agents <= 4 ? launch_tiles_mode<4>(*p, *io, B, mode, g, s) : launch_tiles_mode<8>(*p, *io, B, mode, g, s);
  }
  if (g.group == 8) {
    switch (g.cells_per_lane) {
      case 1: return launch_step<8, 1>(*p, *io, B, mode, s);
      case 2: return launch_step<8, 2>(*p, *io, B, mode, s);
      case 3: return launch_step<8, 3>(*p, *io, B, mode, s);
      default: return launch_step<8, 4>(*p, *io, B, mode, s);
    }
  }
  if (g.group == 16) {
    switch (g.cells_per_lane) {
      case 1: return launch_step<16, 1>(*p, *io, B, mode, s);
      case 2: return launch_step<16, 2>(*p, *io, B, mode, s);
      case 3: return launch_step<16, 3>(*p, *io, B, mode, s);
      case 4: return launch_step<16, 4>(*p, *io, B, mode, s);
      case 5: return launch_step<16, 5>(*p, *io, B, mode, s);
      case 6: return launch_step<16, 6>(*p, *io, B, mode, s);
      case 7: return launch_step<16, 7>(*p, *io, B, mode, s);
      default: return launch_step<16, 8>(*p, *io, B, mode, s);
    }
  }
  switch (g.cells_per_lane) {
    case 1: return launch_step<32, 1>(*p, *io, B, mode, s);
    case 2: return launch_step<32, 2>(*p, *io, B, mode, s);
    case 4: return launch_step<32, 4>(*p, *io, B, mode, s);
    default: return launch_step<32, 8>(*p, *io, B, mode, s);
  }
}

}
}

extern "C" {

int frz_wildfire_step(const FrzWildfireParams* params, const FrzWildfireBuffers* io, int32_t parallel_envs, void* stream) {
  if (io != nullptr && io->actions == nullptr) {
    frz::set_error("frz_wildfire_step: actions is NULL");
    return FRZ_ERR_NULL;
  }
  return frz::dispatch(params, io, parallel_envs, frz::kStep, stream);
}

int frz_wildfire_step_host(const FrzWildfireParams* params, const FrzWildfireBuffers* io, int32_t parallel_envs,
                           const FrzHostStep* host, void* stream) {
  if (params == nullptr || io == nullptr || io->actions == nullptr || io->control == nullptr || io->rewards == nullptr) {
    frz::set_error("frz_wildfire_step_host: NULL params / buffers");
    return FRZ_ERR_NULL;
  }
  if (io->field_uniforms != nullptr || io->agent_uniforms != nullptr) {
    frz::set_error("frz_wildfire_step_host: injected uniforms are not supported on the pipelined host path");
    return FRZ_ERR_UNSUPPORTED;
  }
  const size_t HW = size_t(params->height) * params->width, A = size_t(params->num_agents);
  const frz::HostArrays arrays{io->actions, io->rewards, io->terminated, io->truncated, io->control, params->num_agents,
                                 params, sizeof(FrzWildfireParams), io, sizeof(FrzWildfireBuffers)};
  return frz::run_host_pipeline(
      "frz_wildfire_step_host", host, arrays, parallel_envs, static_cast<cudaStream_t>(stream),
      [&](int first, int count, FrzControl* control, cudaStream_t slice_stream) {
        FrzWildfireParams p = *params;
        p.env_offset += first;
        FrzWildfireBuffers slice = *io;
        const size_t e = size_t(first);
        slice.fires += e * HW;
        slice.intensity += e * HW;
        slice.fuel += e * HW;
        slice.suppressants += e * A;
        slice.capacity += e * A;
        slice.equipment += e * A;
        slice.actions += e * A * 2;
        slice.rewards += e * A;
        slice.cumulative_rewards += e * A;
        slice.terminated += e;
        slice.truncated += e;
        slice.num_moves += e;
        slice.num_burnouts += e;
        slice.burnouts += e;
        slice.putouts += e;
        slice.env_task_count += e;
        slice.agent_task_count += e * A;
        slice.action_mask += e * A * size_t(io->mask_stride);
        slice.self_obs += e * A * 4;
        slice.task_obs += e * HW * 4;
        slice.control = control;
        return frz::dispatch(&p, &slice, count, frz::kStep, slice_stream);
      });
}

int frz_wildfire_tile_random_layout(const FrzWildfireParams* params, uint32_t* streams, int8_t* destinations) {
  frz::Geometry g;
  if (params == nullptr || streams == nullptr || destinations == nullptr) {
    frz::set_error("frz_wildfire_tile_random_layout: NULL argument");
    return -FRZ_ERR_NULL;
  }
  if (!frz::pick_geometry(*params, &g) || !frz::small_grid(*params) || g.group != 8) {
    frz::set_error("frz_wildfire_tile_random_layout: H=%d W=%d A=%d is not a small grid", params->height, params->width,
                   params->num_agents);
    return -FRZ_ERR_SHAPE;
  }
  FrzWildfireParams folded;
  frz::Derived derived;
  frz::fold_configuration(*params, g.group, g.cells_per_lane, &folded, &derived);
  const frz::SmallRandomLayout layout = frz::small_random_layout(
      params->height * params->width, params->num_agents, g.group, g.cells_per_lane, derived.spare_lanes_feed_agents != 0);
  for (int i = 0; i < layout.calls; ++i) {
    streams[i] = layout.stream[i];
    for (int j = 0; j < 4; ++j) destinations[4 * i + j] = layout.dest[i][j];
  }
  return layout.calls;
}

int frz_wildfire_refresh(const FrzWildfireParams* params, const FrzWildfireBuffers* io, int32_t parallel_envs,
                         void* stream) {
  return frz::dispatch(params, io, parallel_envs, frz::kRefresh, stream);
}

int frz_wildfire_reset(const FrzWildfireParams* params, const FrzWildfireBuffers* io, int32_t parallel_envs,
                       const uint8_t* env_mask, void* stream) {
  if (params == nullptr || io == nullptr || io->init_fires == nullptr || io->control == nullptr) {
    frz::set_error("frz_wildfire_reset: NULL params / buffers");
    return FRZ_ERR_NULL;
  }
  if (parallel_envs <= 0) {
    frz::set_error("frz_wildfire_reset: parallel_envs=%d", parallel_envs);
    return FRZ_ERR_SHAPE;
  }
  const int HW = params->height * params->width;
  const size_t total = size_t(parallel_envs) * (HW > params->num_agents ? HW : params->num_agents);
  const int grid = frz::persistent_grid(int((total + 255) / 256 < (1u << 20) ? (total + 255) / 256 : (1u << 20)), 16);
  frz::wildfire_restore_kernel<<<grid, 256, 0, static_cast<cudaStream_t>(stream)>>>(*params, *io, parallel_envs, env_mask);
  const int status = frz::check_launch("wildfire_restore_kernel");
  if (status != FRZ_OK) return status;
  return frz::dispatch(params, io, parallel_envs, frz::kRefresh, stream);
}

int frz_wildfire_sample_actions(const FrzWildfireParams* params, const FrzWildfireBuffers* io, int32_t parallel_envs,
                                uint64_t sampler_seed, void* stream) {
  if (params == nullptr || io == nullptr || io->actions == nullptr || io->control == nullptr) {
    frz::set_error("frz_wildfire_sample_actions: NULL params / buffers");
    return FRZ_ERR_NULL;
  }
  const int total = parallel_envs * params->num_agents;
  const int grid = frz::persistent_grid((total + 255) / 256, 8);
  frz::wildfire_sample_kernel<<<grid, 256, 0, static_cast<cudaStream_t>(stream)>>>(*params, *io, parallel_envs, sampler_seed);
  return frz::check_launch("wildfire_sample_kernel");
}

}
```

### free_range_zoo_b200/envs/wildfire/env/wildfire.py

```python
from __future__ import annotations

import ctypes
from typing import Any, Callable, Dict, List, Optional, Tuple

import numpy as np
import torch

from free_range_zoo_b200 import _lib
from free_range_zoo_b200.envs.wildfire.env.structures.state import WildfireState
from free_range_zoo_b200.utils.containers import (LazyDict, ObservationDict, jagged_from_padded,
                                                  jagged_indices_from_mask)
from free_range_zoo_b200.utils.conversions import batched_aec_to_batched_parallel
from free_range_zoo_b200.utils import compact
from free_range_zoo_b200.utils.env import AutoresetRows, BatchedAECEnv
from free_range_zoo_b200.utils.spaces import BatchedActionSpace, Space


def parallel_env(wrappers: List[Callable] = [], **kwargs):
    env = raw_env(**kwargs)
    for wrapper in wrappers:
        env = wrapper(env)
    return batched_aec_to_batched_parallel(env)


def env(wrappers: List[Callable] = [], **kwargs):
    environment = raw_env(**kwargs)
    for wrapper in wrappers:
        environment = wrapper(environment)
    return environment


def _np(tensor, dtype):
    return np.ascontiguousarray(torch.as_tensor(tensor).detach().cpu().numpy().astype(dtype))


def spread_lut(weights) -> np.ndarray:
    w = _np(weights, np.float32).reshape(3, 3)
    taps = (w[0, 1], w[1, 0], w[1, 2], w[2, 1])
    lut = np.zeros(16, dtype=np.float32)
    for pattern in range(16):
        acc = np.float32(0.0)
        for bit, tap in enumerate(taps):
            if pattern >> bit & 1:
                acc = np.float32(acc + tap)
        lut[pattern] = acc
    return lut


def flatten_configuration(config, max_steps, show_bad_actions: bool, env_offset: int = 0):
    fc, ac, rc, sc = config.fire_config, config.agent_config, config.reward_config, config.stochastic_config
    H, W = int(config.grid_height), int(config.grid_width)
    A = int(ac.agents.shape[0])
    equipment_states = _np(ac.equipment_states, np.float32)
    E = equipment_states.shape[0]
    capacities = _np(ac.possible_capacities, np.float32)
    if H * W > _lib.MAX_CELLS or A > _lib.MAX_AGENTS or E > _lib.MAX_EQUIPMENT or len(capacities) > _lib.MAX_CAPACITIES:
        raise ValueError(f'wildfire configuration exceeds the engine limits: H*W={H * W} (<= {_lib.MAX_CELLS}), '
                         f'agents={A} (<= {_lib.MAX_AGENTS}), equipment states={E}, capacities={len(capacities)}')

    p = _lib.WildfireParams()
    p.height, p.width, p.num_agents = H, W, A
    p.num_fire_states = int(fc.num_fire_states)
    p.num_equipment_states = E
    p.num_capacities = len(capacities)
    p.max_steps = 2**31 - 1 if max_steps is None else int(max_steps)
    flags = 0
    for name, bit in _lib.WF_FLAGS.items():
        if getattr(sc, name):
            flags |= bit
    if rc.burnout_penalty_scaled:
        flags |= _lib.WF_BURNOUT_SCALED
    if rc.localize_putouts:
        flags |= _lib.WF_LOCALIZE_PUTOUTS
    if show_bad_actions:
        flags |= _lib.WF_SHOW_BAD_ACTIONS
    p.flags = flags
    p.env_offset = env_offset
    p.p_increase = fc.intensity_increase_probability
    p.p_burnout = fc.burnout_probability
    p.p_decrease = fc.intensity_decrease_probability
    p.decrease_bonus = fc.extra_power_decrease_bonus
    p.p_random_ignition = config.fire_random_spread_weight
    p.spread_lut[:] = spread_lut(config.fire_spread_weights).tolist()
    p.p_suppressant_decrease = ac.suppressant_decrease_probability
    p.p_refill = ac.suppressant_refill_probability
    p.p_repair = ac.repair_probability
    p.p_degrade = ac.degrade_probability
    p.p_critical = ac.critical_error_probability
    p.p_tank_switch = ac.tank_switch_probability
    cumulative = np.cumsum(_np(ac.capacity_probabilities, np.float32), dtype=np.float32)
    for i in range(len(capacities)):
        p.capacity_cum[i] = cumulative[i]
        p.capacity_value[i] = capacities[i]
    for e in range(E):
        p.equipment_capacity_bonus[e] = equipment_states[e, 0]
        p.equipment_power_bonus[e] = equipment_states[e, 1]
    p.bad_attack_penalty = rc.bad_attack_penalty
    p.burnout_penalty = rc.burnout_penalty
    p.termination_reward = rc.termination_reward
    p.termination_kappa = rc.termination_kappa
    positions = _np(ac.agents, np.int32)
    power = _np(ac.fire_reduction_power, np.float32)
    for a in range(A):
        p.agent_y[a], p.agent_x[a], p.agent_power[a] = int(positions[a, 0]), int(positions[a, 1]), float(power[a])

    words = (H * W + 31) // 32
    ys, xs = np.divmod(np.arange(H * W), W)
    attack_range = _np(ac.attack_range, np.float32)
    range_mask = np.zeros((A, E, words), dtype=np.uint32)
    for a in range(A):
        chebyshev = np.maximum(np.abs(positions[a, 0] - ys), np.abs(positions[a, 1] - xs)).astype(np.float32)
        for e in range(E):
            reach = np.float32(attack_range[a] + equipment_states[e, 2])
            for c in np.nonzero(chebyshev <= reach)[0]:
                range_mask[a, e, c >> 5] |= np.uint32(1 << (c & 31))
    return p, _np(rc.fire_rewards, np.float32).reshape(-1), _np(fc.ignition_temp, np.int32).reshape(-1), range_mask


def compact_bounds(config) -> Dict[str, int]:
    H, W, fc = int(config.grid_height), int(config.grid_width), config.fire_config
    max_fire_type = max(int(fc.max_fire_type), int(torch.as_tensor(fc.fire_types).abs().max()))
    return dict(task_obs=max(H - 1, W - 1, max_fire_type, int(fc.num_fire_states) - 1),
                agent_task_count=H * W)


def transpose_range_mask(range_mask: np.ndarray, cells: int) -> np.ndarray:
    agents, states, _ = range_mask.shape
    cell_agents = np.zeros((states, cells), dtype=np.uint32)
    for a in range(agents):
        for e in range(states):
            for c in range(cells):
                if int(range_mask[a, e, c >> 5]) >> (c & 31) & 1:
                    cell_agents[e, c] |= np.uint32(1 << a)
    return cell_agents


class raw_env(BatchedAECEnv):

    metadata = {"render.modes": ["human", "rgb_array"], "name": "wildfire_v0", "is_parallelizable": True,
                "render_fps": 2}

    @torch.no_grad()
    def __init__(self, *args, observe_other_suppressant: bool = False, observe_other_power: bool = False,
                 show_bad_actions: bool = False, step_kernel: str = 'auto', **kwargs) -> None:
        super().__init__(*args, **kwargs)
        if step_kernel not in ('auto', 'tiles', 'groups'):
            raise ValueError(f"step_kernel must be 'auto', 'tiles' or 'groups', not {step_kernel!r}")
        self._step_kernel = step_kernel
        self.observe_other_suppressant = observe_other_suppressant
        self.observe_other_power = observe_other_power
        self.show_bad_actions = show_bad_actions

        A = int(self.agent_config.agents.shape[0])
        self.possible_agents = tuple(f"firefighter_{i}" for i in range(1, A + 1))
        self.agents = self.possible_agents
        self.agent_name_mapping = dict(zip(self.possible_agents, range(A)))
        self.max_x, self.max_y = int(self.config.grid_width), int(self.config.grid_height)
        self.ignition_temp = self.fire_config.ignition_temp
        self.agent_observation_bounds = (self.max_y, self.max_x, self.agent_config.max_fire_reduction_power,
                                         self.agent_config.suppressant_states)
        self.fire_observation_bounds = (self.max_y, self.max_x, self.fire_config.max_fire_type,
                                        self.fire_config.num_fire_states)
        other_columns = [0, 1] + ([2] if observe_other_power else []) + ([3] if observe_other_suppressant else [])
        self._other_columns = torch.tensor(other_columns, device=self.device)
        self._other_agents = {
            agent: torch.tensor([i for i in range(A) if i != index], dtype=torch.int64, device=self.device)
            for agent, index in self.agent_name_mapping.items()
        }

        self._params, cell_reward, cell_ignition, range_mask = flatten_configuration(
            self.config, self.max_steps, show_bad_actions, self.env_offset)
        self._params.flags |= {'auto': 0, 'tiles': _lib.WF_KERNEL_TILES, 'groups': _lib.WF_KERNEL_GROUPS}[step_kernel]
        B, HW, dev = self.parallel_envs, self.max_y * self.max_x, self.device
        self._allocate_runtime(A)
        self._mask_stride = (HW + 3) // 4 * 4
        i32, f32 = torch.int32, torch.float32
        self._state = WildfireState(
            fires=torch.zeros((B, self.max_y, self.max_x), dtype=i32, device=dev),
            intensity=torch.zeros((B, self.max_y, self.max_x), dtype=i32, device=dev),
            fuel=torch.zeros((B, self.max_y, self.max_x), dtype=i32, device=dev),
            agents=torch.as_tensor(self.agent_config.agents, dtype=i32).to(dev),
            suppressants=torch.ones((B, A), dtype=f32, device=dev),
            capacity=torch.ones((B, A), dtype=f32, device=dev),
            equipment=torch.ones((B, A), dtype=i32, device=dev),
        )
        self._initial = self._state.clone()
        self.num_burnouts = torch.zeros(B, dtype=i32, device=dev)
        self._burnouts = torch.zeros(B, dtype=i32, device=dev)
        self._putouts = torch.zeros(B, dtype=i32, device=dev)
        self._action_mask = torch.zeros((B, A, self._mask_stride), dtype=torch.uint8, device=dev)
        self._self_obs = torch.zeros((B, A, 4), dtype=f32, device=dev)
        self._task_obs = torch.full((B, HW, 4), _lib.PAD, dtype=i32, device=dev)
        self._cell_reward = torch.from_numpy(cell_reward).to(dev)
        self._cell_ignition = torch.from_numpy(cell_ignition).to(dev)
        self._range_mask = torch.from_numpy(range_mask.view(np.int32)).to(dev)
        self._cell_agents = torch.from_numpy(transpose_range_mask(range_mask, HW).view(np.int32)).to(dev)
        self._uniforms = (None, None)
        self._io = self._bind_buffers()

    def _bind_buffers(self) -> _lib.WildfireBuffers:
        s, init = self._state, self._initial
        io = _lib.WildfireBuffers()
        tensors = dict(
            fires=s.fires, intensity=s.intensity, fuel=s.fuel, suppressants=s.suppressants, capacity=s.capacity,
            equipment=s.equipment, init_fires=init.fires, init_intensity=init.intensity, init_fuel=init.fuel,
            init_suppressants=init.suppressants, init_capacity=init.capacity, init_equipment=init.equipment,
            actions=self._actions, rewards=self._rewards, cumulative_rewards=self._cumulative,
            terminated=self._terminated, truncated=self._truncated, num_moves=self.num_moves,
            num_burnouts=self.num_burnouts, burnouts=self._burnouts, putouts=self._putouts,
            env_task_count=self.environment_task_count, agent_task_count=self._agent_task_count,
            action_mask=self._action_mask, self_obs=self._self_obs, task_obs=self._task_obs,
            cell_reward=self._cell_reward, cell_ignition=self._cell_ignition, range_mask=self._range_mask,
            cell_agents=self._cell_agents,
            control=self._control, field_uniforms=self._uniforms[0], agent_uniforms=self._uniforms[1])
        for name, tensor in tensors.items():
            if tensor is not None:
                assert tensor.is_contiguous() and tensor.device == self.device, name
            setattr(io, name, _lib.pointer(tensor))
        io.mask_stride = self._mask_stride
        io.mask_words = self._range_mask.shape[-1]
        self._bound = tensors
        return io


    @torch.no_grad()
    def reset(self, seed=None, options: Dict[str, Any] = None) -> None:
        super().reset(seed=seed, options=options)
        self._params.max_steps = self._horizon()
        fc, ac, dev = self.fire_config, self.agent_config, self.device
        init = self._initial
        if options is not None and options.get('initial_state') is not None:
            given = options['initial_state']
            if len(given) != self.parallel_envs:
                raise ValueError("Initial state must have the same number of environments as the parallel environments")
            for name in ('fires', 'intensity', 'fuel', 'suppressants', 'capacity', 'equipment'):
                getattr(init, name).copy_(getattr(given, name).to(dev))
        else:
            lit = torch.as_tensor(fc.lit, dtype=torch.bool).to(dev)
            fire_types = torch.as_tensor(fc.fire_types, dtype=torch.int32).to(dev)
            ignition = torch.as_tensor(fc.ignition_temp, dtype=torch.int32).to(dev)
            fires = torch.where(lit, fire_types, -fire_types)
            init.fires.copy_(fires.unsqueeze(0).expand_as(init.fires))
            init.intensity.copy_(torch.where(lit, ignition, torch.zeros_like(ignition)).unsqueeze(0).expand_as(init.fires))
            init.fuel.copy_(torch.where(fires != 0, int(fc.initial_fuel), 0).unsqueeze(0).expand_as(init.fires))
            init.suppressants.fill_(float(ac.initial_suppressant))
            init.capacity.fill_(float(ac.initial_capacity))
            init.equipment.fill_(int(ac.initial_equipment_state))
        self._state.initial_state = init
        self.fire_reduction_power = ac.fire_reduction_power
        self.suppressant_states = ac.suppressant_states
        self._reset_masked(None)
        self._snapshot_reset()
        self.infos = dict({agent: {} for agent in self.agents}, burnouts=self._burnouts, putouts=self._putouts)
        self._rebind_outputs()
        if self.log_directory is not None:
            self._log_environment(reset=True)

    def _reset_masked(self, mask: Optional[torch.Tensor]) -> None:
        _lib.check(self._lib.frz_wildfire_reset(ctypes.byref(self._params), ctypes.byref(self._io), self.parallel_envs,
                                                _lib.pointer(mask), self._stream()), 'frz_wildfire_reset')

    @classmethod
    def _autoreset_rows(cls) -> AutoresetRows:
        state = ('fires', 'intensity', 'fuel', 'suppressants', 'capacity', 'equipment')
        return AutoresetRows(
            init={name: f'init_{name}' for name in state},
            snapshot=('action_mask', 'self_obs', 'task_obs', 'env_task_count', 'agent_task_count'),
            zero=('cumulative_rewards', 'terminated', 'truncated', 'num_moves', 'num_burnouts'),
            overwritten=('rewards', 'burnouts', 'putouts'),
            static=tuple(f'init_{name}' for name in state) + (
                'actions', 'cell_reward', 'cell_ignition', 'range_mask', 'cell_agents', 'control', 'field_uniforms',
                'agent_uniforms'),
            agents_with_tasks=True)


    def step_environment(self) -> Tuple[Dict[str, torch.Tensor], Dict[str, torch.Tensor], Dict[str, Dict]]:
        _lib.check(self._lib.frz_wildfire_step(ctypes.byref(self._params), ctypes.byref(self._io), self.parallel_envs,
                                               self._stream()), 'frz_wildfire_step')
        return self._reward_views, self.terminations, self.infos

    def _host_entry(self):
        return self._lib.frz_wildfire_step_host

    def _refresh(self) -> None:
        _lib.check(self._lib.frz_wildfire_refresh(ctypes.byref(self._params), ctypes.byref(self._io),
                                                  self.parallel_envs, self._stream()), 'frz_wildfire_refresh')

    def _observation_download(self):
        dense = dict(self_obs=self._self_obs, agent_task_count=self._agent_task_count)
        ragged = dict(task_obs=(self._task_obs, 1), action_mask=(self._action_mask, len(self.possible_agents)))
        return dense, ragged

    def _compact_schema(self):
        A, p = len(self.possible_agents), self._params
        bounds = compact_bounds(self.config)
        fill = torch.tensor([[float(p.agent_y[a]), float(p.agent_x[a]), p.agent_power[a], 0.0] for a in range(A)],
                            dtype=torch.float32)
        return compact.Schema(capacity=self.max_y * self.max_x, mask_groups=A, arrays=[
            compact.rows('task_obs', self._task_obs, bound=bounds['task_obs']),
            compact.mask('action_mask', self._action_mask, groups=A),
            compact.dense('self_obs', self._self_obs, columns=(3, 1), fill=fill),
            compact.dense('agent_task_count', self._agent_task_count, bound=bounds['agent_task_count']),
        ])

    def update_actions(self) -> None:
        self._refresh()

    def update_observations(self) -> None:
        self._refresh()
        self.update_observation_views()

    def inject_uniforms(self, field: Optional[torch.Tensor], agent: Optional[torch.Tensor]) -> None:
        self._uniforms = (None if field is None else field.to(self.device, torch.float32).contiguous(),
                          None if agent is None else agent.to(self.device, torch.float32).contiguous())
        self._io = self._bind_buffers()

    def sample_actions(self, sampler_seed: int = 2026) -> torch.Tensor:
        _lib.check(self._lib.frz_wildfire_sample_actions(ctypes.byref(self._params), ctypes.byref(self._io),
                                                         self.parallel_envs, ctypes.c_uint64(sampler_seed),
                                                         self._stream()), 'frz_wildfire_sample_actions')
        return self._actions


    def _log_snapshot(self) -> Dict[str, torch.Tensor]:
        s = self._state
        return dict(super()._log_snapshot(), fires=s.fires, intensity=s.intensity, fuel=s.fuel,
                    suppressants=s.suppressants, capacity=s.capacity, equipment=s.equipment,
                    action_mask=self._action_mask, burnouts=self._burnouts, putouts=self._putouts)

    def _log_state_columns(self, host) -> Dict[str, Any]:
        from free_range_zoo_b200.utils.logging_tap import nested
        B = self.parallel_envs
        columns = {name: [nested(host[name][b]) for b in range(B)]
                   for name in ('fires', 'intensity', 'fuel', 'suppressants', 'capacity', 'equipment')}
        columns['agents'] = [str(torch.as_tensor(self.agent_config.agents).tolist())] * B
        return columns

    def _log_mappings(self, host, agent_index: int):
        from free_range_zoo_b200.utils.logging_tap import index_list
        counts = host['env_task_count']
        slots = np.arange(host['action_mask'].shape[2])[None, :] < counts[:, None]
        allowed = slots if self.show_bad_actions else (host['action_mask'][:, agent_index] != 0) & slots
        return [index_list(row) for row in allowed], [index_list(row) for row in slots]

    def _log_extra_columns(self, host, reset: bool) -> Dict[str, Any]:
        B = self.parallel_envs
        return {'burnouts': [None] * B if reset else host['burnouts'].tolist(),
                'putouts': [None] * B if reset else host['putouts'].tolist()}


    @property
    def action_mask(self) -> torch.Tensor:
        return self._action_mask[:, :, :self.max_y * self.max_x]

    @property
    def task_store(self) -> torch.Tensor:
        return jagged_from_padded(self._task_obs, self.environment_task_count, torch.int64)

    def update_observation_views(self) -> None:
        B = self.parallel_envs
        tasks = LazyDict({'tasks': lambda: self.task_store})
        self.observations = {}
        for agent, index in self.agent_name_mapping.items():
            others, columns = self._other_agents[agent], self._other_columns
            self.observations[agent] = ObservationDict(
                {
                    'self': self._self_obs[:, index],
                    'others': (lambda o=others, c=columns: self._self_obs[:, o][:, :, c]),
                    'tasks': (lambda: tasks['tasks']),
                    'tasks_padded': self._task_obs,
                    'task_count': self.environment_task_count,
                    'action_mask': self.action_mask[:, index],
                },
                batch_size=[B],
                device=self.device,
            )
        good = {a: (lambda i=i: jagged_indices_from_mask(self.action_mask[:, i] != 0))
                for a, i in self.agent_name_mapping.items()}
        every = LazyDict({'all': lambda: jagged_indices_from_mask(
            torch.arange(self.max_y * self.max_x, device=self.device).unsqueeze(0) < self.environment_task_count.unsqueeze(1))})
        lit_steps = lambda: torch.arange(self.max_y * self.max_x, device=self.device).unsqueeze(0) < \
            self.environment_task_count.unsqueeze(1)
        if self.show_bad_actions:
            self.agent_action_mapping = LazyDict({a: (lambda: every['all']) for a in self.agents})
            self.agent_bad_actions = LazyDict({
                a: (lambda i=i: jagged_indices_from_mask((self.action_mask[:, i] == 0) & lit_steps()))
                for a, i in self.agent_name_mapping.items()
            })
        else:
            self.agent_action_mapping = LazyDict(good)
            self.agent_bad_actions = {a: None for a in self.agents}
        self.agent_observation_mapping = LazyDict({a: (lambda: every['all']) for a in self.agents})


    @torch.no_grad()
    def action_space(self, agent: str) -> BatchedActionSpace:
        if self.show_bad_actions:
            counts = self.environment_task_count
        else:
            counts = self._agent_task_count[:, self.agent_name_mapping[agent]]
        slots = torch.arange(self.max_y * self.max_x + 1, device=self.device, dtype=torch.int32).unsqueeze(0)
        starts = torch.where(slots == counts.unsqueeze(1), -1, 0).to(torch.int32)
        return BatchedActionSpace(starts, counts + 1)

    @torch.no_grad()
    def observation_space(self, agent: str) -> List[Space]:
        agent_high, fire_high = self.agent_observation_bounds, self.fire_observation_bounds
        other_high = tuple(agent_high[i] for i in self._other_columns.tolist())
        A = len(self.agents)

        def single(num_tasks: int) -> Space:
            return Space.Dict({
                'self': Space.Box(low=[0] * 4, high=agent_high),
                'others': Space.Tuple([Space.Box(low=[0] * len(other_high), high=other_high) for _ in range(A - 1)]),
                'tasks': Space.Tuple([Space.Box(low=[0] * 4, high=fire_high) for _ in range(num_tasks)]),
            })

        cache: Dict[int, Space] = {}
        return [cache.setdefault(n, single(n)) for n in self.environment_task_count.tolist()]
```

### free_range_zoo_b200/utils/env.py

```python
from __future__ import annotations

import ctypes
import math
from abc import ABC, abstractmethod
from typing import Any, Dict, List, NamedTuple, Optional, Tuple

import torch

from free_range_zoo_b200 import _lib
from free_range_zoo_b200.utils import compact
from free_range_zoo_b200.utils.configuration import Configuration
from free_range_zoo_b200.utils.containers import ObservationDict
from free_range_zoo_b200.utils.selector import AgentSelector


HOST_STEP_MAX_DEFAULT_CHUNKS = 5


class AutoresetRows(NamedTuple):
    init: Dict[str, str]
    snapshot: Tuple[str, ...]
    zero: Tuple[str, ...]
    overwritten: Tuple[str, ...]
    static: Tuple[str, ...]
    agents_with_tasks: bool


class _DeviceBound:

    def __init__(self, library, device: torch.device):
        self._library, self._index = library, device.index

    def __getattr__(self, name):
        entry, index = getattr(self._library, name), self._index

        def call(*args):
            if torch.cuda.current_device() == index:
                return entry(*args)
            with torch.cuda.device(index):
                return entry(*args)

        self.__dict__[name] = call
        return call


def _seed_to_u64(seed) -> int:
    if seed is None:
        return int(torch.randint(0, 2**62, (1, )).item())
    if isinstance(seed, torch.Tensor):
        seed = seed.flatten().tolist()
    if isinstance(seed, (list, tuple)):
        folded = 0x9E3779B97F4A7C15
        for value in seed:
            folded = ((folded ^ (int(value) & 0xFFFFFFFFFFFFFFFF)) * 0x100000001B3) & 0xFFFFFFFFFFFFFFFF
        return folded
    return int(seed) & 0xFFFFFFFFFFFFFFFF


class BatchedAECEnv(ABC):

    metadata: Dict[str, Any] = {}

    def __init__(
        self,
        *args,
        configuration: Configuration = None,
        max_steps: int = 1,
        parallel_envs: int = 1,
        device: torch.device = torch.device('cuda'),
        render_mode: str | None = None,
        log_directory: str = None,
        single_seeding: bool = False,
        buffer_size: int = 0,
        override_initialization_check: bool = False,
        env_offset: int = 0,
        detach_outputs: bool = False,
        autoreset: bool = False,
        **kwargs,
    ):
        device = torch.device(device)
        if device.type != 'cuda':
            raise RuntimeError(f'free_range_zoo_b200 runs on CUDA devices only (got device={device}); '
                               'there is no CPU fallback -- use the reference implementation on CPU.')
        if device.index is None:
            device = torch.device('cuda', torch.cuda.current_device())
        if log_directory is not None and str(log_directory).startswith(('postgres', 'mysql')):
            raise NotImplementedError('the asynchronous logging tap writes CSV files or sqlite:// databases; '
                                      f'no driver for {log_directory!r} is available')
        self.parallel_envs = int(parallel_envs)
        self.max_steps = max_steps
        self.device = device
        self.render_mode = render_mode
        self.log_directory = log_directory
        self.override_initialization_check = override_initialization_check
        self.single_seeding = single_seeding
        self.log_description = None
        self.logger = None
        self.env_offset = int(env_offset)
        self.detach_outputs = detach_outputs
        self.autoreset = bool(autoreset)
        if self.autoreset and log_directory is not None:
            raise ValueError('autoreset restarts environments on the device inside the step, which the logging tap does not '
                             'record; autoreset=True needs log_directory=None')

        if configuration is not None:
            self.config = configuration
            for key, value in vars(configuration).items():
                if hasattr(value, 'validate') and not isinstance(value, torch.Tensor):
                    setattr(self, key, value)

        self._lib = _DeviceBound(_lib.library(), self.device)
        self._tap = None
        self._control = torch.zeros(8, dtype=torch.int64, device=self.device)
        self._seed_value = None
        self._graph = None

    def __del__(self):
        handle = getattr(self, '_host_events', None)
        if handle is not None:
            try:
                self._lib.frz_host_pipeline_destroy(handle)
            except Exception:
                pass
            self._host_events = None


    def generator_state_dict(self) -> Dict[str, int]:
        block = self.control_block()
        return {'seed': block['seed'], 'step': block['step'], 'env_offset': self.env_offset}

    def load_generator_state_dict(self, state: Dict[str, int]) -> None:
        if int(state['env_offset']) != self.env_offset:
            raise ValueError(f"the checkpoint was taken with env_offset={int(state['env_offset'])}, this environment has "
                             f'env_offset={self.env_offset}: its environments would continue on other random streams')
        self._seed_value = int(state['seed'])
        _lib.check(self._lib.frz_control_restore(self._control.data_ptr(), ctypes.c_uint64(int(state['seed'])),
                                                 ctypes.c_uint64(int(state['step'])), self._stream()),
                   'frz_control_restore')
        self._refresh()
        self._mid_cycle = False
        self._rebind_outputs()


    @property
    def num_agents(self) -> int:
        return len(self.agents)

    @property
    def max_num_agents(self) -> int:
        return len(self.possible_agents)

    @property
    def unwrapped(self) -> 'BatchedAECEnv':
        return self

    @property
    def terminated(self) -> torch.Tensor:
        if self.autoreset:
            return self._autoreset_flags[1].view(torch.bool)
        return self._terminated.view(torch.bool)

    @property
    def truncated(self) -> torch.Tensor:
        if self.autoreset:
            return self._autoreset_flags[2].view(torch.bool)
        return self._truncated.view(torch.bool)

    @property
    def episode_statistics(self) -> Dict[str, torch.Tensor]:
        if not self.autoreset:
            raise RuntimeError('episode_statistics is recorded by the autoreset: construct the environment with autoreset=True')
        flags = self._autoreset_flags.view(torch.bool)
        return {'done': flags[0], 'terminated': flags[1], 'truncated': flags[2], 'return': self._episode_return,
                'length': self._episode_length}

    @property
    def finished(self) -> torch.Tensor:
        return torch.logical_or(self.terminated, self.truncated)

    @property
    def agent_task_count(self) -> torch.Tensor:
        return self._agent_task_count.t()

    @property
    def rewards(self) -> Dict[str, torch.Tensor]:
        if self._mid_cycle:
            return {agent: self._zero_rewards for agent in self.agents}
        return self._reward_views


    def _allocate_runtime(self, num_agents: int) -> None:
        B, A, dev = self.parallel_envs, num_agents, self.device
        self._actions = torch.zeros((B, A, 2), dtype=torch.int32, device=dev)
        self._rewards = torch.zeros((B, A), dtype=torch.float32, device=dev)
        self._cumulative = torch.zeros((B, A), dtype=torch.float32, device=dev)
        self._terminated = torch.zeros(B, dtype=torch.uint8, device=dev)
        self._truncated = torch.zeros(B, dtype=torch.uint8, device=dev)
        self.num_moves = torch.zeros(B, dtype=torch.int32, device=dev)
        self.environment_task_count = torch.zeros(B, dtype=torch.int32, device=dev)
        self._agent_task_count = torch.zeros((B, A), dtype=torch.int32, device=dev)
        self._zero_rewards = torch.zeros(B, dtype=torch.float32, device=dev)
        if self.autoreset:
            self._autoreset_flags = torch.zeros((3, B), dtype=torch.uint8, device=dev)
            self._episode_return = torch.zeros((B, A), dtype=torch.float32, device=dev)
            self._episode_length = torch.zeros(B, dtype=torch.int32, device=dev)
            self._autoreset_list = torch.zeros(B, dtype=torch.int32, device=dev)
            self._autoreset_count = torch.zeros(1, dtype=torch.int32, device=dev)
            self._autoreset_scratch = torch.zeros(2, dtype=torch.int32, device=dev)

    def _stream(self) -> ctypes.c_void_p:
        return _lib.stream_handle(self.device)

    def _horizon(self) -> int:
        return 2**31 - 1 if self.max_steps is None else int(self.max_steps)


    @torch.no_grad()
    def reset(self, seed=None, options: Optional[Dict[str, Any]] = None) -> None:
        options = options or {}
        if options.get('max_steps') is not None:
            self.max_steps = options['max_steps']
        self._log_label = options.get('log_label')
        self.log_description = options.get('log_description')

        if options.get('skip_seeding'):
            if self._seed_value is None:
                raise ValueError("Seed must be set before skipping seeding is possible")
        else:
            self._seed_value = _seed_to_u64(seed)
        self.seeds = torch.full((self.parallel_envs, ), self._seed_value & 0x7FFFFFFF, dtype=torch.int32,
                                device=self.device)
        _lib.check(self._lib.frz_control_init(self._control.data_ptr(), ctypes.c_uint64(self._seed_value), self._stream()),
                   'frz_control_init')

        self.agents = self.possible_agents
        self.infos = {agent: {} for agent in self.agents}
        self._reward_views = {a: self._rewards[:, i] for i, a in enumerate(self.agents)}
        self._cumulative_rewards = {a: self._cumulative[:, i] for i, a in enumerate(self.agents)}
        terminated, truncated = self.terminated, self.truncated
        self.terminations = {a: terminated for a in self.agents}
        self.truncations = {a: truncated for a in self.agents}
        self.actions = {a: self._actions[:, i] for i, a in enumerate(self.agents)}
        self._agent_slot = {a: i for i, a in enumerate(self.agents)}
        self._mid_cycle = False

        self.agent_selector = AgentSelector(self.agents)
        self.agent_selection = self.agent_selector.reset()

    @torch.no_grad()
    def reset_batches(self, batch_indices, seed=None, options: Optional[Dict[str, Any]] = None) -> None:
        mask = torch.zeros(self.parallel_envs, dtype=torch.uint8, device=self.device)
        mask[torch.as_tensor(batch_indices, device=self.device, dtype=torch.int64)] = 1
        self._reset_masked(mask)
        if self.autoreset:
            self._autoreset_flags.masked_fill_(mask.bool(), 0)
        self._mid_cycle = False
        self._rebind_outputs()

    @abstractmethod
    def _reset_masked(self, mask: Optional[torch.Tensor]) -> None:
        """Launch the domain's reset kernel for the environments selected by ``mask`` (uint8 [B]; None = all)."""


    @classmethod
    def _autoreset_rows(cls) -> AutoresetRows:
        raise NotImplementedError

    def _snapshot_reset(self) -> None:
        if not self.autoreset:
            return
        B, rows, bound = self.parallel_envs, self._autoreset_rows(), self._bound
        if getattr(self, '_reset_snapshot', None) is None:
            self._reset_snapshot = {name: torch.empty_like(bound[name]) for name in rows.snapshot}
        for name, tensor in self._reset_snapshot.items():
            tensor.copy_(bound[name])
        self._autoreset_flags.zero_()
        pairs = ([(bound[dst], bound[src]) for dst, src in rows.init.items()] +
                 [(bound[name], self._reset_snapshot[name]) for name in rows.snapshot] +
                 [(bound[name], None) for name in rows.zero])
        table = (_lib.AutoresetRow * len(pairs))()
        for at, (dst, src) in enumerate(pairs):
            assert dst.shape[0] == B and dst.is_contiguous() and (src is None or src.shape == dst.shape)
            table[at].dst, table[at].src = dst.data_ptr(), _lib.pointer(src)
            table[at].bytes = dst.numel() * dst.element_size() // B
        block = _lib.Autoreset()
        block.terminated, block.truncated = self._terminated.data_ptr(), self._truncated.data_ptr()
        block.done, block.step_terminated, block.step_truncated = (row.data_ptr() for row in self._autoreset_flags)
        block.cumulative_rewards, block.episode_return = self._cumulative.data_ptr(), self._episode_return.data_ptr()
        block.num_moves, block.episode_length = self.num_moves.data_ptr(), self._episode_length.data_ptr()
        if rows.agents_with_tasks:
            block.agent_task_count = self._agent_task_count.data_ptr()
            block.reset_agent_task_count = self._reset_snapshot['agent_task_count'].data_ptr()
        block.control = self._control.data_ptr()
        block.finished, block.finished_count = self._autoreset_list.data_ptr(), self._autoreset_count.data_ptr()
        block.scratch = self._autoreset_scratch.data_ptr()
        block.rows, block.row_count = table, len(pairs)
        block.num_agents = self._cumulative.shape[1]
        self._autoreset_block = (block, table)

    def _autoreset_launch(self) -> None:
        if self.autoreset:
            _lib.check(self._lib.frz_autoreset(ctypes.byref(self._autoreset_block[0]), self.parallel_envs, self._stream()),
                       'frz_autoreset')


    @abstractmethod
    def step_environment(self) -> Tuple[Dict[str, torch.Tensor], Dict[str, torch.Tensor], Dict[str, Dict]]:
        """Launch the domain's fused step kernel; returns (rewards, terminations, infos) views."""

    @abstractmethod
    def update_actions(self) -> None:
        """Refresh task counts / action masks from the current state (already done inside the fused step)."""

    @abstractmethod
    def update_observations(self) -> None:
        """Refresh observations from the current state (already done inside the fused step)."""

    @abstractmethod
    def action_space(self, agent: str):
        """Per-environment action spaces of ``agent`` (a lazily materialised ``Space.Vector``)."""

    @abstractmethod
    def observation_space(self, agent: str):
        """Per-environment observation spaces of ``agent``."""

    @torch.no_grad()
    def step(self, actions: torch.Tensor) -> None:
        self._actions[:, self._agent_slot[self.agent_selection]].copy_(actions, non_blocking=True)
        self._mid_cycle = True
        if self.agent_selector.is_last():
            self._advance()
        self.agent_selection = self.agent_selector.next()

    @torch.no_grad()
    def step_all(self, actions: Optional[torch.Tensor] = None) -> None:
        if actions is not None and actions.data_ptr() != self._actions.data_ptr():
            self._actions.copy_(actions, non_blocking=True)
        self._advance()


    def _host_entry(self):
        raise NotImplementedError

    def _host_pipeline(self, chunks: Optional[int]):
        B, A = self.parallel_envs, len(self.possible_agents)
        if chunks is None:
            chunks = max(1, min(HOST_STEP_MAX_DEFAULT_CHUNKS, B // 12288))
        chunks = max(1, min(int(chunks), _lib.MAX_CHUNKS))
        cached = getattr(self, '_host_state', None)
        if cached is not None and cached['chunks'] == chunks:
            return cached
        state = dict(
            chunks=chunks,
            rewards=self._rewards.cpu().pin_memory(),
            done=torch.stack([self._terminated, self._truncated]).cpu().pin_memory(),
            controls=torch.zeros((chunks, 8), dtype=torch.int64, device=self.device),
            streams=[torch.cuda.Stream(self.device) for _ in range(chunks)],
            main=torch.cuda.Stream(self.device),
            packed=torch.zeros((B, A, 2), dtype=torch.int16, device=self.device),
        )
        if getattr(self, '_host_events', None) is None:
            handle = ctypes.c_void_p()
            _lib.check(self._lib.frz_host_pipeline_create(ctypes.byref(handle)), 'frz_host_pipeline_create')
            self._host_events = handle
        handles = (ctypes.c_void_p * chunks)(*[stream.cuda_stream for stream in state['streams']])
        block = _lib.HostStep()
        block.rewards = state['rewards'].data_ptr()
        block.terminated = state['done'][0].data_ptr()
        block.truncated = state['done'][1].data_ptr()
        block.chunk_controls = state['controls'].data_ptr()
        block.streams = ctypes.cast(handles, ctypes.POINTER(ctypes.c_void_p))
        block.chunks = chunks
        block.packed_actions = state['packed'].data_ptr()
        block.pipeline = self._host_events
        done = state['done'].view(torch.bool)
        state.update(handles=handles, block=block, terminated=done[0], truncated=done[1])
        self._host_state = state
        return state


    def _observation_download(self) -> Tuple[Dict[str, torch.Tensor], Dict[str, Tuple[torch.Tensor, int]]]:
        raise NotImplementedError

    def _gather_state(self):
        state = getattr(self, '_gather', None)
        if state is not None:
            return state
        B, dev = self.parallel_envs, self.device
        dense, ragged = self._observation_download()
        arrays = (_lib.GatherArray * max(1, len(ragged)))()
        packed, layout = {}, {}
        for at, (name, (tensor, groups)) in enumerate(ragged.items()):
            capacity = tensor.shape[2] if tensor.dim() >= 3 and groups > 1 else tensor.shape[1]
            row_shape = tuple(tensor.shape[3:] if groups > 1 else tensor.shape[2:])
            row_bytes = tensor.element_size() * math.prod(row_shape)
            packed[name] = torch.empty(tensor.numel(), dtype=tensor.dtype, device=dev)
            arrays[at].src, arrays[at].dst = tensor.data_ptr(), packed[name].data_ptr()
            arrays[at].row_bytes, arrays[at].capacity, arrays[at].groups = row_bytes, capacity, groups
            layout[name] = (groups, row_shape, row_bytes // tensor.element_size())
        state = dict(
            dense=dense, ragged=ragged, arrays=arrays, packed=packed, layout=layout,
            offsets=torch.zeros(B + 1, dtype=torch.int32, device=dev),
            scratch=torch.zeros((B + 1023) // 1024 + 1, dtype=torch.int32, device=dev),
            host_counts=torch.zeros(B, dtype=torch.int32).pin_memory(),
            host_offsets=torch.zeros(B + 1, dtype=torch.int32).pin_memory(),
            host_dense={name: torch.empty(tensor.shape, dtype=tensor.dtype).pin_memory() for name, tensor in dense.items()},
            host_packed={name: torch.empty(tensor.numel(), dtype=tensor.dtype).pin_memory() for name, tensor in packed.items()},
        )
        self._gather = state
        return state

    def _enqueue_gather(self, state) -> None:
        _lib.check(self._lib.frz_gather_live_rows(self.environment_task_count.data_ptr(), self.parallel_envs,
                                                  state['offsets'].data_ptr(), state['scratch'].data_ptr(), state['arrays'],
                                                  len(state['ragged']), self._stream()), 'frz_gather_live_rows')
        state['host_counts'].copy_(self.environment_task_count, non_blocking=True)
        state['host_offsets'].copy_(state['offsets'], non_blocking=True)
        for name, tensor in state['dense'].items():
            state['host_dense'][name].copy_(tensor, non_blocking=True)

    def _finish_gather(self, state) -> Dict[str, Any]:
        B = self.parallel_envs
        total = int(state['host_offsets'][B])
        moved = state['host_counts'].numel() * 4 + state['host_offsets'].numel() * 4
        moved += sum(t.numel() * t.element_size() for t in state['host_dense'].values())
        out: Dict[str, Any] = {'counts': state['host_counts'], 'offsets': state['host_offsets'], 'total': total}
        out.update(state['host_dense'])
        for name, device_rows in state['packed'].items():
            groups, row_shape, row_elements = state['layout'][name]
            live = total * groups * row_elements
            host_rows = state['host_packed'][name][:live]
            if live:
                host_rows.copy_(device_rows[:live], non_blocking=True)
            moved += live * device_rows.element_size()
            out[name] = host_rows.view((total * groups, ) + row_shape) if row_shape else host_rows
        torch.cuda.current_stream(self.device).synchronize()
        out['bytes'] = moved
        return out

    def _compact_schema(self) -> compact.Schema:
        raise NotImplementedError

    def _compact_download(self) -> compact.CompactDownload:
        download = getattr(self, '_compact', None)
        if download is None or download.key != self.max_steps:
            download = compact.CompactDownload(self._compact_schema(), self.environment_task_count, key=self.max_steps)
            self._compact = download
        return download

    def _enqueue_compact(self) -> compact.CompactDownload:
        download = self._compact_download()
        _lib.check(self._lib.frz_observe_compact(ctypes.byref(download.block), self.parallel_envs, self._stream()),
                   'frz_observe_compact')
        return download

    @torch.no_grad()
    def gather_observations(self, compact: bool = False) -> Dict[str, Any]:
        with torch.cuda.device(self.device):
            if compact:
                download = self._enqueue_compact()
                torch.cuda.current_stream(self.device).synchronize()
                return download.result()
            state = self._gather_state()
            self._enqueue_gather(state)
            torch.cuda.current_stream(self.device).synchronize()
            return self._finish_gather(state)

    @torch.no_grad()
    def step_host(self, host_actions: torch.Tensor, chunks: Optional[int] = None, observations: bool | str = False
                  ) -> Tuple[torch.Tensor, ...]:
        if not (isinstance(observations, bool) or (isinstance(observations, str) and observations == 'compact')):
            raise ValueError(f"observations must be False, True or 'compact', not {observations!r}")
        B, A = self.parallel_envs, len(self.possible_agents)
        if (host_actions.device.type != 'cpu' or host_actions.dtype not in (torch.int32, torch.int16, torch.int8)
                or not host_actions.is_contiguous() or tuple(host_actions.shape) != (B, A, 2)
                or not host_actions.is_pinned()):
            raise ValueError(f'step_host expects a page-locked contiguous int32 / int16 / int8 CPU tensor of shape {(B, A, 2)} '
                             '(torch.empty(..., dtype=torch.int32).pin_memory())')
        state = self._host_pipeline(chunks)
        state['block'].actions = host_actions.data_ptr()
        state['block'].action_format = {torch.int32: _lib.HOST_ACTIONS_I32, torch.int16: _lib.HOST_ACTIONS_I16,
                                        torch.int8: _lib.HOST_ACTIONS_I8}[host_actions.dtype]
        current, main = torch.cuda.current_stream(self.device), state['main']
        main.wait_stream(current)
        _lib.check(self._host_entry()(ctypes.byref(self._params), ctypes.byref(self._io), B,
                                      ctypes.byref(state['block']), ctypes.c_void_p(main.cuda_stream)), 'step_host')
        with torch.cuda.stream(main):
            self._autoreset_launch()
        current.wait_stream(main)
        self._mid_cycle = False
        self._rebind_outputs()
        if self.log_directory is not None:
            self._log_environment()
        if not observations:
            main.synchronize()
            return state['rewards'], state['terminated'], state['truncated']
        if observations == 'compact':
            with torch.cuda.stream(main):
                download = self._enqueue_compact()
            main.synchronize()
            return state['rewards'], state['terminated'], state['truncated'], download.result()
        with torch.cuda.stream(main):
            gather = self._gather_state()
            self._enqueue_gather(gather)
            main.synchronize()
            packed = self._finish_gather(gather)
        return state['rewards'], state['terminated'], state['truncated'], packed

    def _advance(self) -> None:
        _, _, infos = self.step_environment()
        self._autoreset_launch()
        self.infos = infos
        self._mid_cycle = False
        self._rebind_outputs()
        if self.log_directory is not None:
            self._log_environment()


    def _log_environment(self, reset: bool = False) -> None:
        if self._tap is None:
            from free_range_zoo_b200.utils.logging_tap import LoggingTap
            if str(self.log_directory).startswith('sqlite://'):
                from free_range_zoo_b200.utils.sql_tap import SqliteSink
                sink = SqliteSink(self.log_directory, self.metadata['name'], self.parallel_envs)
                self._tap = LoggingTap(self.log_directory, self.parallel_envs, self.device, self._log_snapshot,
                                       self._log_records, sink=sink, agents=self.possible_agents)
            else:
                self._tap = LoggingTap(self.log_directory, self.parallel_envs, self.device, self._log_snapshot,
                                       self._log_columns,
                                       override_initialization_check=self.override_initialization_check)
        self._tap.capture(reset, self.log_description, getattr(self, '_log_label', None))

    def flush_logs(self) -> None:
        if self._tap is not None:
            self._tap.flush()

    def _log_snapshot(self) -> Dict[str, torch.Tensor]:
        return dict(actions=self._actions, rewards=self._rewards, num_moves=self.num_moves, terminated=self._terminated,
                    truncated=self._truncated, env_task_count=self.environment_task_count,
                    agent_task_count=self._agent_task_count)

    def _log_columns(self, host: Dict[str, Any], reset: bool) -> Dict[str, Any]:
        from free_range_zoo_b200.utils.logging_tap import nested
        B = self.parallel_envs
        columns = dict(self._log_state_columns(host))
        finished = (host['terminated'] != 0) | (host['truncated'] != 0)
        for index, agent in enumerate(self.possible_agents):
            columns[f'{agent}_action'] = [None] * B if reset else [nested(host['actions'][b, index]) for b in range(B)]
            columns[f'{agent}_rewards'] = [None] * B if reset else host['rewards'][:, index].astype(float).tolist()
        columns['step'] = [-1] * B if reset else host['num_moves'].tolist()
        columns['complete'] = [None] * B if reset else finished.tolist()
        for index, agent in enumerate(self.possible_agents):
            action_map, observation_map = self._log_mappings(host, index)
            columns[f'{agent}_action_map'] = action_map
            columns[f'{agent}_observation_map'] = observation_map
        columns.update(self._log_extra_columns(host, reset))
        return columns

    def _log_records(self, host: Dict[str, Any], reset: bool) -> Dict[str, Any]:
        state = dict(self._log_state_columns(host))
        state.update({name: cells for name, cells in self._log_extra_columns(host, reset).items()
                      if name not in ('burnouts', 'putouts')})
        agents = {}
        for index, agent in enumerate(self.possible_agents):
            action_map, observation_map = self._log_mappings(host, index)
            agents[agent] = dict(reward=host['rewards'][:, index], action_field=host['actions'][:, index, 1],
                                 task_field=host['actions'][:, index, 0], action_map=action_map,
                                 observation_map=observation_map)
        return dict(timestep=host['num_moves'], state=state, agents=agents)

    def _log_state_columns(self, host) -> Dict[str, Any]:
        raise NotImplementedError

    def _log_mappings(self, host, agent_index: int):
        raise NotImplementedError

    def _log_extra_columns(self, host, reset: bool) -> Dict[str, Any]:
        return {}

    def _rebind_outputs(self) -> None:
        self.update_observation_views()
        if self.detach_outputs:
            self._reward_views = {a: self._rewards[:, i].clone() for i, a in enumerate(self.agents)}
            terminated, truncated = self.terminated.clone(), self.truncated.clone()
            self.terminations = {a: terminated for a in self.agents}
            self.truncations = {a: truncated for a in self.agents}

    @abstractmethod
    def update_observation_views(self) -> None:
        """Build ``self.observations`` (dict agent -> ObservationDict) as views of the device buffers."""

    @torch.no_grad()
    def observe(self, agent: str) -> ObservationDict:
        return self.observations[agent]

    @torch.no_grad()
    def state(self):
        return self._state

    def last(self, observe: bool = True):
        agent = self.agent_selection
        observation = self.observe(agent) if observe else None
        return (observation, self._cumulative_rewards[agent], self.terminations[agent], self.truncations[agent],
                self.infos[agent])


    def control_block(self) -> Dict[str, int]:
        raw = self._control.cpu().numpy().tobytes()
        block = _lib.Control.from_buffer_copy(raw)
        return {name: getattr(block, name) for name, _ in _lib.Control._fields_ if name != 'reserved'}

    def check_errors(self) -> None:
        word = self.control_block()['error_word']
        if word:
            self._control.view(torch.int32)[7] = 0
            reasons = [text for bit, text in _lib.FAULT_NAMES.items() if word & bit]
            raise ValueError('invalid actions were submitted: ' + '; '.join(reasons))


    def capture_graph(self, sample: bool = False, sampler_seed: int = 2026, steps: int = 1) -> None:
        if self.log_directory is not None:
            raise RuntimeError('graph replays bypass the logging tap; capture_graph needs log_directory=None')
        torch.cuda.synchronize(self.device)
        saved = {name: tensor.clone() for name, tensor in self._bound.items()
                 if tensor is not None and not name.startswith('init_')}
        autoreset = [self._autoreset_flags, self._episode_return, self._episode_length] if self.autoreset else []
        saved_autoreset = [tensor.clone() for tensor in autoreset]
        side = torch.cuda.Stream(self.device)
        side.wait_stream(torch.cuda.current_stream(self.device))
        with torch.cuda.stream(side):
            if sample:
                self.sample_actions(sampler_seed)
            self.step_environment()
            self._autoreset_launch()
        torch.cuda.current_stream(self.device).wait_stream(side)
        torch.cuda.synchronize(self.device)
        for name, tensor in saved.items():
            self._bound[name].copy_(tensor)
        for tensor, copy in zip(autoreset, saved_autoreset):
            tensor.copy_(copy)
        del saved
        torch.cuda.synchronize(self.device)
        graph = torch.cuda.CUDAGraph()
        with torch.cuda.graph(graph):
            for _ in range(max(1, int(steps))):
                if sample:
                    self.sample_actions(sampler_seed)
                self.step_environment()
                self._autoreset_launch()
        self._graph = graph

    def replay(self) -> None:
        self._graph.replay()
        self._mid_cycle = False
        if self.detach_outputs:
            self._rebind_outputs()

    def sample_actions(self, sampler_seed: int = 2026) -> torch.Tensor:
        raise NotImplementedError
```

Baseline: 665.3 million.

## Fuse multi-step wildfire rollout into one persistent kernel with per-pair step flags

Adds a rollout mode to the wildfire step kernel. One launch runs several steps with in-kernel action sampling, and fine-grained release/acquire flags let each env pair advance to the next step as soon as its previous step finishes, instead of waiting for a grid-wide launch boundary. It is used by default in capture_graph when sampling is on. The aim is to remove per-step launch and sampling-kernel overhead and the tail idle time between steps. The cost is spin-waiting with a stall fault, ring-buffer bookkeeping, and added complexity and deadlock risk if CTAs are not all resident.

Measured after the change: 307.6 million, median of 6. 0.462x the previous value.

```diff
diff --git a/__graft_entry__.py b/__graft_entry__.py
--- a/__graft_entry__.py
+++ b/__graft_entry__.py
@@ -15,7 +15,7 @@
     assert os.path.exists(path), path
     from free_range_zoo_b200 import _lib
     lib = _lib.library()
-    missing = [name for header in ('frz.h', 'frz_obs.h', 'frz_autoreset.h') for name in _lib.exported_symbols(header)
+    missing = [name for header in ('frz.h', 'frz_obs.h', 'frz_autoreset.h', 'frz_rollout.h') for name in _lib.exported_symbols(header)
                if not hasattr(lib, name)]
     if missing:
         raise RuntimeError(f'libfrz.so does not export {missing}')
diff --git a/free_range_zoo_b200/_lib.py b/free_range_zoo_b200/_lib.py
--- a/free_range_zoo_b200/_lib.py
+++ b/free_range_zoo_b200/_lib.py
@@ -22,6 +22,7 @@
     0x2: 'cybersecurity attack / movement target outside [0, num_nodes)',
     0x4: 'a non-present cybersecurity agent acted while show_bad_actions=False',
     0x8: 'rideshare passenger table overflow',
+    0x10: 'a rollout task waited too long for the step before it (FRZ_FAULT_ROLLOUT_STALL, include/frz_rollout.h)',
 }
 
 
@@ -211,6 +212,10 @@
                                          C.c_void_p]
     lib.frz_observe_compact.argtypes = [C.POINTER(ObsDownload), C.c_int32, C.c_void_p]
     lib.frz_autoreset.argtypes = [C.POINTER(Autoreset), C.c_int32, C.c_void_p]
+    lib.frz_wildfire_rollout_scratch_bytes.argtypes = [C.POINTER(WildfireParams), C.c_int32, C.c_int32]
+    lib.frz_wildfire_rollout_scratch_bytes.restype = C.c_int64
+    lib.frz_wildfire_rollout.argtypes = [C.POINTER(WildfireParams), C.POINTER(WildfireBuffers), C.c_int32, C.c_int32,
+                                         C.c_uint64, C.c_void_p, C.c_void_p]
     if lib.frz_version() != ABI_VERSION:
         raise RuntimeError(f'libfrz.so ABI version {lib.frz_version()} != {ABI_VERSION}; rebuild the library')
     lib.frz_control_restore.argtypes = [C.c_void_p, C.c_uint64, C.c_uint64, C.c_void_p]
diff --git a/free_range_zoo_b200/csrc/frz_common.cuh b/free_range_zoo_b200/csrc/frz_common.cuh
--- a/free_range_zoo_b200/csrc/frz_common.cuh
+++ b/free_range_zoo_b200/csrc/frz_common.cuh
@@ -51,18 +51,21 @@
 
 template <class Kernel>
 int resident_ctas(Kernel kernel, int threads, size_t smem) {
-  static int ctas[kMaxDevices] = {};
-  static size_t smem_of[kMaxDevices] = {};
+  struct Entry {
+    const void* kernel;
+    int device, threads;
+    size_t smem;
+    int ctas;
+  };
+  thread_local std::vector<Entry> cache;
+  const void* key = reinterpret_cast<const void*>(kernel);
   const int device = current_device();
-  const bool cacheable = device >= 0 && device < kMaxDevices;
-  if (cacheable && ctas[device] > 0 && smem_of[device] == smem) return ctas[device];
+  for (const Entry& e : cache)
+    if (e.kernel == key && e.device == device && e.threads == threads && e.smem == smem) return e.ctas;
   int count = 0;
   cudaOccupancyMaxActiveBlocksPerMultiprocessor(&count, kernel, threads, smem);
   if (count < 1) count = 1;
-  if (cacheable) {
-    ctas[device] = count;
-    smem_of[device] = smem;
-  }
+  cache.push_back({key, device, threads, smem, count});
   return count;
 }
 
@@ -206,6 +209,22 @@
   asm volatile("cp.async.bulk.wait_group.read %0;" : : "n"(pending) : "memory");
 }
 __device__ __forceinline__ void fence_async_shared() { asm volatile("fence.proxy.async.shared::cta;" : : : "memory"); }
+__device__ __forceinline__ void bulk_wait_all() { asm volatile("cp.async.bulk.wait_group 0;" : : : "memory"); }
+__device__ __forceinline__ void fence_async_global() { asm volatile("fence.proxy.async.global;" : : : "memory"); }
+
+__device__ __forceinline__ uint32_t ld_acquire(const uint32_t* address) {
+  uint32_t value;
+  asm volatile("ld.acquire.gpu.global.u32 %0, [%1];" : "=r"(value) : "l"(address) : "memory");
+  return value;
+}
+__device__ __forceinline__ uint32_t ld_relaxed(const uint32_t* address) {
+  uint32_t value;
+  asm volatile("ld.relaxed.gpu.global.u32 %0, [%1];" : "=r"(value) : "l"(address) : "memory");
+  return value;
+}
+__device__ __forceinline__ void st_release(uint32_t* address, uint32_t value) {
+  asm volatile("st.release.gpu.global.u32 [%0], %1;" : : "l"(address), "r"(value) : "memory");
+}
 
 
 enum Publish { kPublishNothing = 0, kPublishRefresh = 1, kPublishStep = 2 };
diff --git a/free_range_zoo_b200/csrc/frz_wildfire.cu b/free_range_zoo_b200/csrc/frz_wildfire.cu
--- a/free_range_zoo_b200/csrc/frz_wildfire.cu
+++ b/free_range_zoo_b200/csrc/frz_wildfire.cu
@@ -3,6 +3,7 @@
 
 #include "frz_common.cuh"
 #include "frz_host.cuh"
+#include "frz_rollout.h"
 
 namespace frz {
 namespace {
@@ -11,7 +12,7 @@
 #define FRZ_WF_THREADS 256
 #endif
 constexpr int kThreads = FRZ_WF_THREADS;
-enum Mode { kStep = 0, kRefresh = 1 };
+enum Mode { kStep = 0, kRefresh = 1, kRollout = 2 };
 
 template <int NW>
 __device__ __forceinline__ uint32_t word_at(const uint32_t (&words)[NW], int index) {
@@ -111,13 +112,59 @@
   int32_t t_capacity_cum[FRZ_MAX_CAPACITIES];
   int32_t almost_state, burned_state;
   int32_t cells;
+  uint32_t rollout_scratch_lo, rollout_scratch_hi, sampler_seed_lo, sampler_seed_hi;
+  int32_t rollout_steps, rollout_pairs;
+  __host__ __device__ uint32_t* scratch() const { return reinterpret_cast<uint32_t*>((uint64_t(rollout_scratch_hi) << 32) | rollout_scratch_lo); }
+  __host__ __device__ uint64_t seed() const { return (uint64_t(sampler_seed_hi) << 32) | sampler_seed_lo; }
 };
+
+constexpr int kRolloutHeader = 4;
+constexpr uint32_t kRolloutSkipped = 4u;
+constexpr uint32_t kRolloutSpinLimit = 1u << 22;
+
+__device__ __forceinline__ int2 sample_action(const Philox& sampler, uint64_t genv, uint64_t step, int agent, int n) {
+  const uint4 r = sampler(uint32_t(genv), uint32_t(step), 0xC0000000u | uint32_t(agent),
+                          uint32_t(step >> 32) ^ uint32_t(genv >> 32));
+  const int k = min(int(u01(r.x) * float(n + 1)), n);
+  return make_int2(k, k == n ? -1 : 0);
+}
+
+__device__ __forceinline__ void finish_rollout(FrzControl* control, const Derived& derived, unsigned fault_bits) {
+  __shared__ unsigned s_fault;
+  if (threadIdx.x == 0) s_fault = 0;
+  __syncthreads();
+  if (fault_bits) atomicOr(&s_fault, fault_bits);
+  __syncthreads();
+  if (threadIdx.x == 0) {
+    if (s_fault) atomicOr(&control->error_word, s_fault);
+    __threadfence();
+    const unsigned arrived = atomicAdd(&control->ctas_done, 1u) + 1u;
+    if (arrived == gridDim.x) {
+      __threadfence();
+      volatile uint32_t* const ring = derived.scratch() + kRolloutHeader;
+      uint32_t alive = control->alive, agents = control->agents_with_tasks, executed = 0;
+      for (int s = 0; s < derived.rollout_steps && (alive & 3u) == 3u; ++s, ++executed) {
+        alive = ring[4 * s];
+        agents = ring[4 * s + 1];
+      }
+      for (int i = 0; i < 4 * derived.rollout_steps; ++i) ring[i] = 0u;
+      if (executed > 0) {
+        control->alive = alive;
+        control->agents_with_tasks = agents;
+        control->step += executed;
+      }
+      derived.scratch()[0] += uint32_t(derived.rollout_steps);
+      control->ctas_done = 0u;
+    }
+  }
+}
 
 template <int G, int CPL, int MODE, bool INJECTED, bool BULK>
 __global__ void __launch_bounds__(kThreads, (G * CPL > 128) ? 1 : FRZ_WF_MIN_BLOCKS)
 wildfire_step_kernel(const __grid_constant__ FrzWildfireParams p, const __grid_constant__ FrzWildfireBuffers io,
                      const __grid_constant__ Derived derived, const int B) {
-  constexpr int mode = MODE;
+  constexpr bool rollout = MODE == kRollout;
+  constexpr int mode = rollout ? int(kStep) : MODE;
   constexpr int kGroupsPerWarp = 32 / G;
   constexpr int kCells = G * CPL;
   constexpr int NW = (kCells + 31) / 32;
@@ -199,11 +246,12 @@
   __syncthreads();
 
   FrzControl* const control = io.control;
-  const uint64_t step = control->step;
+  const uint64_t step0 = control->step;
+  uint64_t step = step0;
   const uint32_t alive_prev = control->alive;
-  const uint32_t agents_with_tasks = control->agents_with_tasks;
+  uint32_t agents_with_tasks = control->agents_with_tasks;
   const Philox philox(control->seed);
-  const bool skip = (mode == kStep) && ((alive_prev & 3u) != 3u);
+  const bool skip = !rollout && (mode == kStep) && ((alive_prev & 3u) != 3u);
 
   const bool is_agent = sub < A;
   const float base_power = is_agent ? p.agent_power[sub] : 0.f;
@@ -219,6 +267,7 @@
     const auto fetch_state = [&](int pair, uint32_t into) {
       const uint32_t buffer = __shfl_sync(kFullMask, into, 0);
       if (elect_one()) {
+        if (rollout) fence_async_global();
         const uint32_t barrier = s_barriers + 8u * buffer;
         mbarrier_expect_bytes(barrier, uint32_t(kGroupsPerWarp) * 3u * row_bytes);
 #pragma unroll
@@ -231,19 +280,56 @@
         }
       }
       if (is_agent) {
-        const uint32_t at = uint32_t(min(pair + lane / G, B - 1)) * uint32_t(A) + uint32_t(sub);
+        const int env_of_lane = min(pair + lane / G, B - 1);
+        const uint32_t at = uint32_t(env_of_lane) * uint32_t(A) + uint32_t(sub);
         cp_async_4(s_stage, io.suppressants + at);
         cp_async_4(s_stage + 4u * G, io.capacity + at);
         cp_async_4(s_stage + 8u * G, io.equipment + at);
-        if (mode == kStep) cp_async_8(s_stage + 12u * G + 4u * uint32_t(sub), io.actions + 2u * at);
+        if (rollout) cp_async_4(s_stage + 12u * G + 4u * uint32_t(sub), show_bad ? io.env_task_count + env_of_lane : io.agent_task_count + at);
+        else if (mode == kStep) cp_async_8(s_stage + 12u * G + 4u * uint32_t(sub), io.actions + 2u * at);
       }
       cp_async_commit();
     };
     uint32_t buffer = 0u, parities = 0u;
+    const int pair_span = rollout ? derived.rollout_pairs * kGroupsPerWarp : B;
+    const int slot_end = rollout ? derived.rollout_steps * pair_span : B;
+    uint32_t* const ring = derived.scratch() + kRolloutHeader;
+    uint32_t* const done = ring + 4 * derived.rollout_steps;
+    const uint32_t tick = rollout ? derived.scratch()[0] : 0u;
+    const uint32_t all_agents = A >= 32 ? 0xffffffffu : (1u << A) - 1u;
+    bool prefetched = first_env0 < pair_span;
+    bool stalled = false;
+    int pending_pair = -1;
+    uint32_t pending_value = 0u;
+    const auto flush_pending = [&]() {
+      if constexpr (rollout && bulk) {
+        bulk_wait_all();
+        if (pending_pair >= 0) {
+          fence_async_global();
+          st_release(done + pending_pair, pending_value);
+          pending_pair = -1;
+        }
+      }
+    };
+    const auto wait_until = [&](auto ready) {
+      uint32_t sleep = 32u;
+      for (uint32_t polls = 0; !stalled && !ready(); ++polls) {
+        if (polls == kRolloutSpinLimit) {
+          stalled = true;
+          faults |= FRZ_FAULT_ROLLOUT_STALL;
+          break;
+        }
+        __nanosleep(sleep);
+        sleep = min(2u * sleep, 1024u);
+      }
+    };
     if constexpr (kCellsInSmem) {
-      if (bulk && first_env0 < B) fetch_state(first_env0, 0u);
+      if (bulk && first_env0 < pair_span) fetch_state(first_env0, 0u);
     }
-    for (int env0 = first_env0; env0 < B; env0 += gridDim.x * groups_per_cta) {
+    for (int slot = first_env0; slot < slot_end; slot += gridDim.x * groups_per_cta) {
+      const int s = rollout ? slot / pair_span : 0;
+      const int env0 = slot - s * pair_span;
+      const int pair = env0 / kGroupsPerWarp;
       const int env = env0 + lane / G;
       const bool valid = (G == 32) || env < B;
       const int e = valid ? env : B - 1;
@@ -252,6 +338,58 @@
       int* const fires_row = io.fires + cell_row;
       int* const inten_row = io.intensity + cell_row;
       int* const fuel_row = io.fuel + cell_row;
+
+      if constexpr (rollout) {
+        uint32_t prior_alive = alive_prev, prior_agents = agents_with_tasks;
+        if (s > 0 && lane == 0) {
+          const uint32_t* const prior = ring + 4 * (s - 1);
+          prior_alive = ld_relaxed(prior);
+          prior_agents = ld_relaxed(prior + 1);
+          if (prior_alive != 3u || prior_agents != all_agents) {
+            flush_pending();
+            wait_until([&] { return ld_acquire(prior + 2) >= uint32_t(derived.rollout_pairs); });
+            prior_alive = ld_relaxed(prior);
+            prior_agents = ld_relaxed(prior + 1);
+          }
+          if (int(ld_acquire(done + pair) - (tick + uint32_t(s))) < 0) {
+            flush_pending();
+            wait_until([&] { return int(ld_acquire(done + pair) - (tick + uint32_t(s))) >= 0; });
+          }
+        }
+        __syncwarp();
+        prior_alive = __shfl_sync(kFullMask, prior_alive, 0);
+        agents_with_tasks = __shfl_sync(kFullMask, prior_agents, 0);
+        step = step0 + uint64_t(s);
+        if ((prior_alive & 3u) != 3u) {
+          if constexpr (bulk) {
+            if (prefetched) {
+              mbarrier_wait(s_barriers + 8u * buffer, (parities >> buffer) & 1u);
+              parities ^= 1u << buffer;
+              cp_async_wait_all();
+            }
+          }
+          prefetched = false;
+          if (!(prior_alive & kRolloutSkipped) && valid && is_agent) {
+            const int n = show_bad ? io.env_task_count[e] : io.agent_task_count[agent_at];
+            reinterpret_cast<int2*>(const_cast<int32_t*>(io.actions))[agent_at] =
+                sample_action(Philox(derived.seed()), uint64_t(p.env_offset + e), step, sub, n);
+          }
+          __threadfence();
+          __syncwarp();
+          if (lane == 0) {
+            flush_pending();
+            atomicOr(ring + 4 * s, kRolloutSkipped);
+            __threadfence();
+            atomicAdd(ring + 4 * s + 2, 1u);
+            st_release(done + pair, tick + uint32_t(s) + 1u);
+          }
+          __syncwarp();
+          continue;
+        }
+        if constexpr (bulk) {
+          if (!prefetched) fetch_state(env0, buffer);
+        }
+      }
 
       int cell_regs[3][kCellsInSmem ? 1 : CPL] = {};
       const auto cell = [&](int plane, int i) -> int {
@@ -311,7 +449,19 @@
       bool terminated = false, truncated = false;
 
       const auto prefetch_next = [&]() {
-        if constexpr (kCellsInSmem) {
+        if constexpr (rollout && bulk) {
+          const int next = slot + gridDim.x * groups_per_cta;
+          const int next_s = next / pair_span, next_env0 = next - next_s * pair_span;
+          bool ready = next < slot_end;
+          if (lane == 0) {
+            flush_pending();
+            if (ready && next_s > 0)
+              ready = int(ld_acquire(done + next_env0 / kGroupsPerWarp) - (tick + uint32_t(next_s))) >= 0;
+          }
+          __syncwarp();
+          prefetched = __shfl_sync(kFullMask, ready, 0);
+          if (prefetched) fetch_state(next_env0, buffer ^ 1u);
+        } else if constexpr (kCellsInSmem) {
           const int next_env0 = env0 + gridDim.x * groups_per_cta;
           if (bulk && next_env0 < B) {
             if (lane == 0) bulk_wait_read();
@@ -324,7 +474,14 @@
       if (mode == kStep) {
         int act_k = 0, act_id = -1;
         if (is_agent) {
-          const int2 act = bulk ? staged_action : reinterpret_cast<const int2*>(io.actions)[agent_at];
+          int2 act;
+          if constexpr (rollout) {
+            const int n = bulk ? staged_action.x : (show_bad ? io.env_task_count[e] : io.agent_task_count[agent_at]);
+            act = sample_action(Philox(derived.seed()), uint64_t(p.env_offset + e), step, sub, n);
+            if (valid) reinterpret_cast<int2*>(const_cast<int32_t*>(io.actions))[agent_at] = act;
+          } else {
+            act = bulk ? staged_action : reinterpret_cast<const int2*>(io.actions)[agent_at];
+          }
           act_k = act.x;
           act_id = act.y;
           cumulative = io.cumulative_rewards[agent_at];
@@ -831,13 +988,36 @@
         }
       }
       __syncwarp();
+      if constexpr (rollout) {
+        __threadfence();
+        __syncwarp();
+        const uint32_t task_alive = __reduce_or_sync(kFullMask, alive_bits);
+        const uint32_t task_agents = __reduce_or_sync(kFullMask, agent_bits);
+        alive_bits = agent_bits = 0u;
+        if (lane == 0) {
+          uint32_t* const flags = ring + 4 * s;
+          if (task_alive) atomicOr(flags, task_alive);
+          if (task_agents) atomicOr(flags + 1, task_agents);
+          __threadfence();
+          atomicAdd(flags + 2, 1u);
+          if (bulk) {
+            pending_pair = pair;
+            pending_value = tick + uint32_t(s) + 1u;
+          } else {
+            st_release(done + pair, tick + uint32_t(s) + 1u);
+          }
+        }
+        __syncwarp();
+      }
     }
+    if (rollout && lane == 0) flush_pending();
     if constexpr (kCellsInSmem) {
       if (bulk && lane == 0) bulk_wait_read();
     }
   }
-  finish_launch(control, alive_bits, faults, agent_bits,
-                skip ? kPublishNothing : (mode == kStep ? kPublishStep : kPublishRefresh));
+  if constexpr (rollout) finish_rollout(control, derived, faults);
+  else finish_launch(control, alive_bits, faults, agent_bits,
+                     skip ? kPublishNothing : (mode == kStep ? kPublishStep : kPublishRefresh));
 }
 
 
@@ -884,10 +1064,8 @@
   for (int i = blockIdx.x * blockDim.x + threadIdx.x; i < total; i += gridDim.x * blockDim.x) {
     const int env = i / A, agent = i - env * A;
     const int n = show_bad ? io.env_task_count[env] : io.agent_task_count[i];
-    const uint64_t genv = uint64_t(p.env_offset + env);
-    const uint4 r = philox(uint32_t(genv), uint32_t(step), 0xC0000000u | uint32_t(agent), uint32_t(step >> 32) ^ uint32_t(genv >> 32));
-    const int k = min(int(u01(r.x) * float(n + 1)), n);
-    reinterpret_cast<int2*>(const_cast<int32_t*>(io.actions))[i] = make_int2(k, k == n ? -1 : 0);
+    reinterpret_cast<int2*>(const_cast<int32_t*>(io.actions))[i] =
+        sample_action(philox, uint64_t(p.env_offset + env), step, agent, n);
   }
 }
 
@@ -999,10 +1177,17 @@
   return launch_tiles<MAXA, kStep, false>(p, io, B, g, stream);
 }
 
+struct Rollout {
+  int steps;
+  uint64_t sampler_seed;
+  uint32_t* scratch;
+};
+
 template <int G, int CPL, int MODE, bool INJECTED, bool BULK>
-int launch_variant(const FrzWildfireParams& caller_params, const FrzWildfireBuffers& io, int B, cudaStream_t stream) {
+int launch_variant(const FrzWildfireParams& caller_params, const FrzWildfireBuffers& io, int B, const Rollout* rollout,
+                   cudaStream_t stream) {
   FrzWildfireParams p;
-  Derived derived;
+  Derived derived = {};
   fold_configuration(caller_params, G, CPL, &p, &derived);
   const int groups_per_cta = (kThreads / 32) * (32 / G);
   const size_t smem = (size_t(static_smem_words(G * CPL, p.num_agents, p.num_equipment_states)) +
@@ -1013,29 +1198,64 @@
     if (cudaFuncSetAttribute(kernel, cudaFuncAttributeMaxDynamicSharedMemorySize, int(smem)) != cudaSuccess)
       return check_launch("wildfire smem attribute");
   }
-  const int grid = persistent_grid((B + groups_per_cta - 1) / groups_per_cta, resident_ctas(kernel, kThreads, smem));
-  kernel<<<grid, kThreads, smem, stream>>>(p, io, derived, B);
-  return check_launch("wildfire_step_kernel");
+  if constexpr (MODE == kRollout) {
+    const int pairs = (B + 32 / G - 1) / (32 / G);
+    const int64_t task_ctas = (int64_t(rollout->steps) * pairs + kThreads / 32 - 1) / (kThreads / 32);
+    derived.rollout_scratch_lo = uint32_t(reinterpret_cast<uintptr_t>(rollout->scratch));
+    derived.rollout_scratch_hi = uint32_t(reinterpret_cast<uintptr_t>(rollout->scratch) >> 32);
+    derived.sampler_seed_lo = uint32_t(rollout->sampler_seed);
+    derived.sampler_seed_hi = uint32_t(rollout->sampler_seed >> 32);
+    derived.rollout_steps = rollout->steps;
+    derived.rollout_pairs = pairs;
+    const int grid = persistent_grid(int(task_ctas < (1 << 30) ? task_ctas : (1 << 30)), resident_ctas(kernel, kThreads, smem));
+    cudaLaunchAttribute attribute = {};
+    attribute.id = cudaLaunchAttributeCooperative;
+    attribute.val.cooperative = 1;
+    cudaLaunchConfig_t config = {};
+    config.gridDim = dim3(grid);
+    config.blockDim = dim3(kThreads);
+    config.dynamicSmemBytes = smem;
+    config.stream = stream;
+    config.attrs = &attribute;
+    config.numAttrs = 1;
+    cudaLaunchKernelEx(&config, kernel, p, io, derived, B);
+    return check_launch("wildfire_step_kernel (rollout)");
+  } else {
+    const int grid = persistent_grid((B + groups_per_cta - 1) / groups_per_cta, resident_ctas(kernel, kThreads, smem));
+    kernel<<<grid, kThreads, smem, stream>>>(p, io, derived, B);
+    return check_launch("wildfire_step_kernel");
+  }
 }
 
 template <int G, int CPL, bool BULK>
-int launch_mode(const FrzWildfireParams& p, const FrzWildfireBuffers& io, int B, int mode, cudaStream_t stream) {
-  if (mode != kStep) return launch_variant<G, CPL, kRefresh, false, BULK>(p, io, B, stream);
-  if (io.field_uniforms != nullptr || io.agent_uniforms != nullptr) return launch_variant<G, CPL, kStep, true, BULK>(p, io, B, stream);
-  return launch_variant<G, CPL, kStep, false, BULK>(p, io, B, stream);
+int launch_mode(const FrzWildfireParams& p, const FrzWildfireBuffers& io, int B, int mode, const Rollout* rollout,
+                cudaStream_t stream) {
+  if (mode == kRollout) return launch_variant<G, CPL, kRollout, false, BULK>(p, io, B, rollout, stream);
+  if (mode != kStep) return launch_variant<G, CPL, kRefresh, false, BULK>(p, io, B, nullptr, stream);
+  if (io.field_uniforms != nullptr || io.agent_uniforms != nullptr)
+    return launch_variant<G, CPL, kStep, true, BULK>(p, io, B, nullptr, stream);
+  return launch_variant<G, CPL, kStep, false, BULK>(p, io, B, nullptr, stream);
 }
 
 template <int G, int CPL>
-int launch_step(const FrzWildfireParams& p, const FrzWildfireBuffers& io, int B, int mode, cudaStream_t stream) {
+int launch_step(const FrzWildfireParams& p, const FrzWildfireBuffers& io, int B, int mode, const Rollout* rollout,
+                cudaStream_t stream) {
   if constexpr (cells_in_smem(G, CPL)) {
     const uintptr_t bases = reinterpret_cast<uintptr_t>(io.fires) | reinterpret_cast<uintptr_t>(io.intensity) |
                             reinterpret_cast<uintptr_t>(io.fuel);
-    if ((p.height * p.width) % 4 == 0 && bases % 16 == 0) return launch_mode<G, CPL, true>(p, io, B, mode, stream);
-  }
-  return launch_mode<G, CPL, false>(p, io, B, mode, stream);
-}
-
-int dispatch(const FrzWildfireParams* p, const FrzWildfireBuffers* io, int B, int mode, void* stream) {
+    if ((p.height * p.width) % 4 == 0 && bases % 16 == 0) return launch_mode<G, CPL, true>(p, io, B, mode, rollout, stream);
+  }
+  return launch_mode<G, CPL, false>(p, io, B, mode, rollout, stream);
+}
+
+bool uses_tiles(const FrzWildfireParams& p, const Geometry& g, int B) {
+  return small_grid(p) && g.group == 8 &&
+         ((p.flags & FRZ_WF_KERNEL_TILES) ||
+          (!(p.flags & FRZ_WF_KERNEL_GROUPS) && tiny_grid(p) && B >= kSmallTileMinimumBatch));
+}
+
+int dispatch(const FrzWildfireParams* p, const FrzWildfireBuffers* io, int B, int mode, void* stream,
+             const Rollout* rollout = nullptr) {
   if (p == nullptr || io == nullptr || io->control == nullptr || io->fires == nullptr || io->cell_agents == nullptr ||
       io->range_mask == nullptr) {
     set_error("frz_wildfire: NULL params / buffers");
@@ -1058,36 +1278,39 @@
     }
   }
   cudaStream_t s = static_cast<cudaStream_t>(stream);
-  if (small_grid(*p) && g.group == 8 &&
-      ((p->flags & FRZ_WF_KERNEL_TILES) ||
-       (!(p->flags & FRZ_WF_KERNEL_GROUPS) && tiny_grid(*p) && B >= kSmallTileMinimumBatch))) {
+  if (uses_tiles(*p, g, B)) {
+    if (mode == kRollout) {
+      set_error("frz_wildfire_rollout: H=%d W=%d A=%d B=%d is stepped by the tile kernel, which has no rollout",
+                p->height, p->width, p->num_agents, B);
+      return FRZ_ERR_UNSUPPORTED;
+    }
     return p->num_agents <= 4 ? launch_tiles_mode<4>(*p, *io, B, mode, g, s) : launch_tiles_mode<8>(*p, *io, B, mode, g, s);
   }
   if (g.group == 8) {
     switch (g.cells_per_lane) {
-      case 1: return launch_step<8, 1>(*p, *io, B, mode, s);
-      case 2: return launch_step<8, 2>(*p, *io, B, mode, s);
-      case 3: return launch_step<8, 3>(*p, *io, B, mode, s);
-      default: return launch_step<8, 4>(*p, *io, B, mode, s);
+      case 1: return launch_step<8, 1>(*p, *io, B, mode, rollout, s);
+      case 2: return launch_step<8, 2>(*p, *io, B, mode, rollout, s);
+      case 3: return launch_step<8, 3>(*p, *io, B, mode, rollout, s);
+      default: return launch_step<8, 4>(*p, *io, B, mode, rollout, s);
     }
   }
   if (g.group == 16) {
     switch (g.cells_per_lane) {
-      case 1: return launch_step<16, 1>(*p, *io, B, mode, s);
-      case 2: return launch_step<16, 2>(*p, *io, B, mode, s);
-      case 3: return launch_step<16, 3>(*p, *io, B, mode, s);
-      case 4: return launch_step<16, 4>(*p, *io, B, mode, s);
-      case 5: return launch_step<16, 5>(*p, *io, B, mode, s);
-      case 6: return launch_step<16, 6>(*p, *io, B, mode, s);
-      case 7: return launch_step<16, 7>(*p, *io, B, mode, s);
-      default: return launch_step<16, 8>(*p, *io, B, mode, s);
+      case 1: return launch_step<16, 1>(*p, *io, B, mode, rollout, s);
+      case 2: return launch_step<16, 2>(*p, *io, B, mode, rollout, s);
+      case 3: return launch_step<16, 3>(*p, *io, B, mode, rollout, s);
+      case 4: return launch_step<16, 4>(*p, *io, B, mode, rollout, s);
+      case 5: return launch_step<16, 5>(*p, *io, B, mode, rollout, s);
+      case 6: return launch_step<16, 6>(*p, *io, B, mode, rollout, s);
+      case 7: return launch_step<16, 7>(*p, *io, B, mode, rollout, s);
+      default: return launch_step<16, 8>(*p, *io, B, mode, rollout, s);
     }
   }
   switch (g.cells_per_lane) {
-    case 1: return launch_step<32, 1>(*p, *io, B, mode, s);
-    case 2: return launch_step<32, 2>(*p, *io, B, mode, s);
-    case 4: return launch_step<32, 4>(*p, *io, B, mode, s);
-    default: return launch_step<32, 8>(*p, *io, B, mode, s);
+    case 1: return launch_step<32, 1>(*p, *io, B, mode, rollout, s);
+    case 2: return launch_step<32, 2>(*p, *io, B, mode, rollout, s);
+    case 4: return launch_step<32, 4>(*p, *io, B, mode, rollout, s);
+    default: return launch_step<32, 8>(*p, *io, B, mode, rollout, s);
   }
 }
 
@@ -1172,6 +1395,43 @@
   return layout.calls;
 }
 
+int64_t frz_wildfire_rollout_scratch_bytes(const FrzWildfireParams* params, int32_t parallel_envs, int32_t steps) {
+  frz::Geometry g;
+  if (params == nullptr) {
+    frz::set_error("frz_wildfire_rollout_scratch_bytes: NULL params");
+    return -FRZ_ERR_NULL;
+  }
+  if (parallel_envs <= 0 || steps < 1 || !frz::pick_geometry(*params, &g) ||
+      int64_t(steps) * (int64_t(parallel_envs) + 32) >= (int64_t(1) << 31)) {
+    frz::set_error("frz_wildfire_rollout_scratch_bytes: unsupported B=%d steps=%d H=%d W=%d A=%d", parallel_envs, steps,
+                   params->height, params->width, params->num_agents);
+    return -FRZ_ERR_SHAPE;
+  }
+  if (frz::uses_tiles(*params, g, parallel_envs)) {
+    frz::set_error("frz_wildfire_rollout_scratch_bytes: H=%d W=%d A=%d B=%d is stepped by the tile kernel, which has no "
+                   "rollout", params->height, params->width, params->num_agents, parallel_envs);
+    return -FRZ_ERR_UNSUPPORTED;
+  }
+  const int64_t pairs = (parallel_envs + 32 / g.group - 1) / (32 / g.group);
+  return 4 * (frz::kRolloutHeader + 4 * int64_t(steps) + pairs);
+}
+
+int frz_wildfire_rollout(const FrzWildfireParams* params, const FrzWildfireBuffers* io, int32_t parallel_envs,
+                         int32_t steps, uint64_t sampler_seed, void* scratch, void* stream) {
+  if (params == nullptr || io == nullptr || io->actions == nullptr || scratch == nullptr) {
+    frz::set_error("frz_wildfire_rollout: NULL params / buffers / scratch");
+    return FRZ_ERR_NULL;
+  }
+  if (io->field_uniforms != nullptr || io->agent_uniforms != nullptr) {
+    frz::set_error("frz_wildfire_rollout: injected uniforms are not supported; step with frz_wildfire_step");
+    return FRZ_ERR_UNSUPPORTED;
+  }
+  const int64_t bytes = frz_wildfire_rollout_scratch_bytes(params, parallel_envs, steps);
+  if (bytes < 0) return int(-bytes);
+  const frz::Rollout rollout{steps, sampler_seed, static_cast<uint32_t*>(scratch)};
+  return frz::dispatch(params, io, parallel_envs, frz::kRollout, stream, &rollout);
+}
+
 int frz_wildfire_refresh(const FrzWildfireParams* params, const FrzWildfireBuffers* io, int32_t parallel_envs,
                          void* stream) {
   return frz::dispatch(params, io, parallel_envs, frz::kRefresh, stream);
diff --git a/free_range_zoo_b200/envs/wildfire/env/wildfire.py b/free_range_zoo_b200/envs/wildfire/env/wildfire.py
--- a/free_range_zoo_b200/envs/wildfire/env/wildfire.py
+++ b/free_range_zoo_b200/envs/wildfire/env/wildfire.py
@@ -315,6 +315,23 @@
                           None if agent is None else agent.to(self.device, torch.float32).contiguous())
         self._io = self._bind_buffers()
 
+    def _rollout_launcher(self, steps: int, sampler_seed: int):
+        if self.autoreset or self._uniforms != (None, None):
+            return None
+        size = self._lib.frz_wildfire_rollout_scratch_bytes(ctypes.byref(self._params), self.parallel_envs, steps)
+        if size == -4:
+            return None
+        if size < 0:
+            _lib.check(-size, 'frz_wildfire_rollout_scratch_bytes')
+        scratch = torch.zeros(size // 4, dtype=torch.int32, device=self.device)
+        self._rollout_scratch = scratch
+
+        def launch() -> None:
+            _lib.check(self._lib.frz_wildfire_rollout(ctypes.byref(self._params), ctypes.byref(self._io), self.parallel_envs,
+                                                      steps, ctypes.c_uint64(sampler_seed), scratch.data_ptr(),
+                                                      self._stream()), 'frz_wildfire_rollout')
+        return launch
+
     def sample_actions(self, sampler_seed: int = 2026) -> torch.Tensor:
         _lib.check(self._lib.frz_wildfire_sample_actions(ctypes.byref(self._params), ctypes.byref(self._io),
                                                          self.parallel_envs, ctypes.c_uint64(sampler_seed),
diff --git a/free_range_zoo_b200/utils/env.py b/free_range_zoo_b200/utils/env.py
--- a/free_range_zoo_b200/utils/env.py
+++ b/free_range_zoo_b200/utils/env.py
@@ -76,6 +76,7 @@
         env_offset: int = 0,
         detach_outputs: bool = False,
         autoreset: bool = False,
+        graph_rollout: bool = True,
         **kwargs,
     ):
         device = torch.device(device)
@@ -99,6 +100,7 @@
         self.env_offset = int(env_offset)
         self.detach_outputs = detach_outputs
         self.autoreset = bool(autoreset)
+        self.graph_rollout = bool(graph_rollout)
         if self.autoreset and log_directory is not None:
             raise ValueError('autoreset restarts environments on the device inside the step, which the logging tap does not '
                              'record; autoreset=True needs log_directory=None')
@@ -622,6 +624,19 @@
         if self.log_directory is not None:
             raise RuntimeError('graph replays bypass the logging tap; capture_graph needs log_directory=None')
         torch.cuda.synchronize(self.device)
+        steps = max(1, int(steps))
+        rollout = self._rollout_launcher(steps, sampler_seed) if sample and self.graph_rollout else None
+
+        def enqueue_steps(count: int) -> None:
+            if rollout is not None:
+                rollout()
+                return
+            for _ in range(count):
+                if sample:
+                    self.sample_actions(sampler_seed)
+                self.step_environment()
+                self._autoreset_launch()
+
         saved = {name: tensor.clone() for name, tensor in self._bound.items()
                  if tensor is not None and not name.startswith('init_')}
         autoreset = [self._autoreset_flags, self._episode_return, self._episode_length] if self.autoreset else []
@@ -629,10 +644,7 @@
         side = torch.cuda.Stream(self.device)
         side.wait_stream(torch.cuda.current_stream(self.device))
         with torch.cuda.stream(side):
-            if sample:
-                self.sample_actions(sampler_seed)
-            self.step_environment()
-            self._autoreset_launch()
+            enqueue_steps(1)
         torch.cuda.current_stream(self.device).wait_stream(side)
         torch.cuda.synchronize(self.device)
         for name, tensor in saved.items():
@@ -643,12 +655,11 @@
         torch.cuda.synchronize(self.device)
         graph = torch.cuda.CUDAGraph()
         with torch.cuda.graph(graph):
-            for _ in range(max(1, int(steps))):
-                if sample:
-                    self.sample_actions(sampler_seed)
-                self.step_environment()
-                self._autoreset_launch()
+            enqueue_steps(steps)
         self._graph = graph
+
+    def _rollout_launcher(self, steps: int, sampler_seed: int):
+        return None
 
     def replay(self) -> None:
         self._graph.replay()
diff --git a/include/frz_rollout.h b/include/frz_rollout.h
--- /dev/null
+++ b/include/frz_rollout.h
@@ -0,0 +1,20 @@
+#ifndef FRZ_ROLLOUT_H_
+#define FRZ_ROLLOUT_H_
+
+#include "frz.h"
+
+#ifdef __cplusplus
+extern "C" {
+#endif
+
+#define FRZ_FAULT_ROLLOUT_STALL 0x10u
+
+int64_t frz_wildfire_rollout_scratch_bytes(const FrzWildfireParams* params, int32_t parallel_envs, int32_t steps);
+
+int frz_wildfire_rollout(const FrzWildfireParams* params, const FrzWildfireBuffers* io, int32_t parallel_envs,
+                         int32_t steps, uint64_t sampler_seed, void* scratch, void* stream);
+
+#ifdef __cplusplus
+}
+#endif
+#endif
diff --git a/profiles/time_rollout.py b/profiles/time_rollout.py
--- /dev/null
+++ b/profiles/time_rollout.py
@@ -0,0 +1,85 @@
+import argparse
+import json
+import os
+import statistics
+import subprocess
+import sys
+
+ROOT = os.path.dirname(os.path.dirname(os.path.abspath(__file__)))
+sys.path.insert(0, ROOT)
+
+WORKLOADS = [('wildfire_c4', dict(), 65536), ('wildfire_c4_262144', dict(), 262144)]
+SEED, SAMPLER = 2026, 2026
+
+
+def gpu_description():
+    import torch
+    info = {'gpu': torch.cuda.get_device_name(0)}
+    try:
+        info['power_limit'] = subprocess.run(['nvidia-smi', '--query-gpu=power.limit', '--format=csv,noheader', '-i', '0'],
+                                             capture_output=True, text=True, timeout=30).stdout.strip()
+    except (OSError, subprocess.SubprocessError):
+        info['power_limit'] = 'unknown'
+    return info
+
+
+def main():
+    parser = argparse.ArgumentParser(description=__doc__, formatter_class=argparse.RawDescriptionHelpFormatter)
+    parser.add_argument('--out', default=None)
+    parser.add_argument('--windows', type=int, default=6)
+    parser.add_argument('--replays', type=int, default=40)
+    args = parser.parse_args()
+    import torch
+
+    from free_range_zoo_b200 import presets
+    from free_range_zoo_b200.envs import wildfire_v0
+    rows = []
+    for name, preset_kwargs, B in WORKLOADS:
+        for steps in (5, 10):
+            engines = {}
+            for variant in ('loop', 'rollout'):
+                env = wildfire_v0.parallel_env(parallel_envs=B, max_steps=1 << 30,
+                                               configuration=presets.wildfire_large(**preset_kwargs),
+                                               device=torch.device('cuda:0'), graph_rollout=variant == 'rollout')
+                raw = env.unwrapped
+                env.reset(seed=SEED)
+                raw.capture_graph(sample=True, sampler_seed=SAMPLER, steps=steps)
+                engines[variant] = (env, raw)
+            times = {variant: [] for variant in engines}
+            start, stop = torch.cuda.Event(enable_timing=True), torch.cuda.Event(enable_timing=True)
+            for _ in range(args.windows):
+                for variant, (env, raw) in engines.items():
+                    env.reset(seed=SEED)
+                    for _ in range(2):
+                        raw.replay()
+                    torch.cuda.synchronize()
+                    start.record()
+                    for _ in range(args.replays):
+                        raw.replay()
+                    stop.record()
+                    torch.cuda.synchronize()
+                    times[variant].append(1e3 * start.elapsed_time(stop) / (args.replays * steps))
+            for variant, (_, raw) in engines.items():
+                raw.check_errors()
+            loop_us, rollout_us = statistics.median(times['loop']), statistics.median(times['rollout'])
+            row = dict(workload=name, envs=B, steps_per_launch=steps, loop_us_per_step=loop_us,
+                       rollout_us_per_step=rollout_us, speedup=loop_us / rollout_us,
+                       loop_spread=(max(times['loop']) - min(times['loop'])) / loop_us,
+                       rollout_spread=(max(times['rollout']) - min(times['rollout'])) / rollout_us,
+                       loop_windows_us=times['loop'], rollout_windows_us=times['rollout'])
+            rows.append(row)
+            print(f'{name} S={steps}: loop {loop_us:.2f} us/step, rollout {rollout_us:.2f} us/step, '
+                  f'x{loop_us / rollout_us:.3f}', flush=True)
+            del engines
+            torch.cuda.empty_cache()
+    result = dict(gpu_description(), windows=args.windows, replays=args.replays, rows=rows)
+    text = json.dumps(result, indent=1)
+    if args.out:
+        with open(args.out, 'w') as handle:
+            handle.write(text + '\n')
+    else:
+        print(text)
+
+
+if __name__ == '__main__':
+    main()
```
